# jiahuei/COMIC-Compact-Image-Captioning-with-Attention

Measured on AMD Instinct MI355X. Metric: images/sec (decoder-mode XE training, COMIC-256, InceptionV3 frozen), higher is better.
Workload: dtype bf16; 1 GPU; MS-COCO decoder-mode XE, COMIC-256 (radix-256, 8 heads, tied), InceptionV3 frozen, batch 64/GPU, 224x224x3 (BASELINE configs[1]); per_gpu_batch=64, global_batch=64, image_size=224, feature_map=5x5x2048, decoder_dtype=f32, parallelism=dp1, encoder_group=8, inputs=resident in HBM, 2 distinct image groups in rotation

## Files before the change

### comic-compact-image-captioning-with-attention_amd/_lib.py

```python
import ctypes as C
import os

_HERE = os.path.dirname(os.path.abspath(__file__))
LIB_PATH = os.environ.get('COMIC_HIP_LIB') or os.path.join(_HERE, 'lib', 'libcomic_hip.so')

c_void_p, c_int, c_int32, c_int64, c_float, c_double, c_char_p, c_uint64 = (
    C.c_void_p, C.c_int, C.c_int32, C.c_int64, C.c_float, C.c_double, C.c_char_p, C.c_uint64)


class CnnOp(C.Structure):
    _fields_ = [(n, c_int32) for n in (
        'kind', 'src', 'dst', 'src_coff', 'dst_coff', 'H', 'W', 'Cin', 'Cout', 'KH', 'KW', 'SH', 'SW',
        'PT', 'PL', 'Ho', 'Wo', 'weight', 'relu', 'out_f32', 'src_f32', 'lane', 'tile', 'group', 'flags', 'min_lds')]


class ImageDesc(C.Structure):
    _fields_ = [('offset', C.c_int64), ('in_h', c_int32), ('in_w', c_int32), ('flip', c_int32), ('oy', c_int32),
                ('ox', c_int32), ('sy', C.c_float), ('sx', C.c_float)]


class ConvWeight(C.Structure):
    _fields_ = [('w', c_void_p), ('scale', c_void_p), ('shift', c_void_p), ('w_frag', c_void_p)]


class AttnDesc(C.Structure):
    _fields_ = [(n, c_int32) for n in ('B', 'M', 'D', 'H', 'Cv', 'method', 'prob', 'tied')]


class DecoderDesc(C.Structure):
    _fields_ = [(n, c_int32) for n in (
        'D', 'E', 'A', 'V', 'C', 'Cg', 'H', 'M', 'Cv', 'fm_projection', 'method', 'prob', 'context_layer',
        'init_method', 'start_id', 'end_id')] + [(n, c_float) for n in (
            'keep_in', 'keep_out', 'keep_alpha', 'map_loss_scale')] + [('flags', C.c_uint32),
                                                                       ('length_penalty_weight', c_float),
                                                                       ('cell', c_int32)]


CELLS = {'LSTM': 0, 'LN_LSTM': 1, 'GRU': 2}


(DEC_NO_PERSIST, DEC_NO_PERSIST_BWD, DEC_NO_FUSED_STEP, DEC_NO_SPLIT_ATTN_BWD, DEC_ONE_LANE, DEC_EXACT_GEMM, DEC_STAMPS,
 DEC_NO_BEAM_LOGITS, DEC_NO_LSTM_STREAM) = (1, 2, 4, 8, 16, 32, 64, 128, 256)
DEC_PHASE_FWD, DEC_PHASE_BWD = 512, 1024
DEC_NO_GROUP_GEMM = 2048
DEC_BWD_OWN_ROWS = 4096
DEC_INJECT_TIMEOUT = 8192
CNN_BWD_NO_ACT_FUSION = 2
_DEC_ENV = (('COMIC_PERSIST', '0', DEC_NO_PERSIST), ('COMIC_PERSIST_BWD', '0', DEC_NO_PERSIST_BWD),
            ('COMIC_FUSED_STEP', '0', DEC_NO_FUSED_STEP), ('COMIC_SPLIT_ATTN_BWD', '0', DEC_NO_SPLIT_ATTN_BWD),
            ('COMIC_GRAD_LANES', '0', DEC_ONE_LANE), ('COMIC_SPLIT3', '0', DEC_EXACT_GEMM),
            ('COMIC_PERSIST_STAMPS', '1', DEC_STAMPS), ('COMIC_BEAM_LOGITS', '0', DEC_NO_BEAM_LOGITS),
            ('COMIC_LSTM_STREAM', '0', DEC_NO_LSTM_STREAM), ('COMIC_GROUP_GEMM', '0', DEC_NO_GROUP_GEMM),
            ('COMIC_BWD_OWN_ROWS', '1', DEC_BWD_OWN_ROWS))


def decoder_flags_from_env():
    f = 0
    for name, val, bit in _DEC_ENV:
        if os.environ.get(name, '')[:1] == val:
            f |= bit
    return f


CONV_TILES = 61
WS_TILE = 54
IMG_TILE = 55
CHAIN_TILE = 62
OP_RAW, OP_POOLED_SRC, OP_X3 = 1, 2, 4
OP_CHAIN_LINK = 8
OP_CHAIN_KEEP = 16
IM2COL_CONV_TILES = 12


def is_im2col_tile(tile):
    return tile <= IM2COL_CONV_TILES or 26 <= tile <= 47
PARAM_NAMES = ('W_init', 'K', 'b', 'W_m', 'W_v', 'W_q', 'v', 'ln_g', 'ln_b', 'tau', 'W_a', 'W_o', 'b_o', 'emb', 'cell_ln', 'K_c', 'b_c', 'status')


class DecoderParams(C.Structure):
    _fields_ = [(n, c_void_p) for n in PARAM_NAMES]


class GemmProb(C.Structure):
    _fields_ = [(n, c_void_p) for n in ('A', 'B', 'C', 'bias', 'mask')] + [(n, c_int32) for n in (
        'M', 'N', 'K', 'lda', 'ldb', 'ldc', 'ld_mask')] + [(n, c_float) for n in ('alpha', 'beta', 'keep')] + [
        ('type', c_int32), ('ones_a', c_int32)]


class ConvGrad(C.Structure):
    _fields_ = [('w_master', c_void_p), ('dw', c_void_p), ('dbeta', c_void_p), ('w_bwd', c_void_p),
                ('bwd_tile', c_int32), ('reserved', c_int32)]


P = c_void_p
_SIGS = {
    'comic_last_error': (c_char_p, []),
    'comic_abi_version': (c_int, []),
    'comic_device_count': (c_int, []),
    'comic_pack_conv_weights': (c_int, [P, P, c_int, c_int, c_int, c_int, c_int, P]),
    'comic_fold_bn': (c_int, [P, P, P, c_float, P, P, c_int, P]),
    'comic_cnn_forward': (c_int, [P, c_int, P, P, P, c_int, c_int, P]),
    'comic_cnn_group_args_bytes': (C.c_long, [P, c_int]),
    'comic_cnn_build_group_args': (c_int, [P, c_int, P, P, P, c_int, P]),
    'comic_cnn_forward_grouped': (c_int, [P, c_int, P, P, P, c_int, c_int, P, P]),
    'comic_clip_by_norm': (c_int, [P, P, P, c_int, c_float, c_float, c_float, P, P, P]),
    'comic_cnn_backward_scratch_bytes': (c_int64, [P, c_int, c_int, c_int, c_int]),
    'comic_cnn_backward': (c_int, [P, c_int, P, P, P, P, P, c_int, c_int, c_int, P, c_int64, P, P]),
    'comic_cnn_backward_sched': (c_int, [P, c_int, P, c_int, P, P, P, P, P, P, c_int, c_int, c_int, P, c_int64, P, P, P]),
    'comic_cnn_pack_bwd_filters': (c_int, [P, c_int, P, c_int, P]),
    'comic_cnn_pack_x3_weights': (c_int, [P, P, P, P, P, c_int, P]),
    'comic_cnn_refresh_weights': (c_int, [P, P, c_int64, P, P, P, P, c_int64, P]),
    'comic_cnn_refresh_weights_dtype': (c_int, [P, P, c_int64, P, P, P, P, c_int64, c_int, P]),
    'comic_cnn_pack_frag_weights': (c_int, [P, P, P, c_int, c_int64, P]),
    'comic_crc32c': (C.c_uint32, [P, C.c_size_t, C.c_uint32]),
    'comic_conv2d_bn_relu': (c_int, [P, P, c_int, P, c_int, P, c_int, c_int, P]),
    'comic_gemm_f32': (c_int, [P, P, P, P, c_int, c_int, c_int, c_int, c_int, c_int, c_int, c_int, c_float,
                               c_float, P]),
    'comic_gemm_f32_split3': (c_int, [P, P, P, P, c_int, c_int, c_int, c_int, c_int, c_int, c_int, c_int, c_float,
                                      c_float, P, c_int64, P]),
    'comic_gemm_f32_splitk': (c_int, [P, P, P, P, c_int, c_int, c_int, c_int, c_int, c_int, c_int, c_int, c_float,
                                      c_float, P, c_int64, P]),
    'comic_gemm_group_workspace': (c_int64, [P, c_int]),
    'comic_gemm_group': (c_int, [P, c_int, P, c_int64, P]),
    'comic_embed_fwd': (c_int, [P, P, P, c_int, c_int, c_int, P]),
    'comic_embed_bwd': (c_int, [P, P, P, c_int, c_int, c_int, P]),
    'comic_dropout_apply': (c_int, [P, P, c_float, P, c_int64, P]),
    'comic_dropout_mask': (c_int, [P, c_int64, c_float, c_uint64, c_uint64, P]),
    'comic_dropout_mask_dev': (c_int, [P, c_int64, c_float, P, c_uint64, P]),
    'comic_dropout_masks4_dev': (c_int, [P, P, P, P, P]),
    'comic_image_preprocess': (c_int, [P, P, c_int, P, c_int, c_int, c_int, P]),
    'comic_jpeg_pixels': (c_int, [P, P, c_int, c_int, c_int, c_int, P, P, P]),
    'comic_jpeg_preprocess': (c_int, [P, P, c_int, c_int, P, P, P, P, c_int, c_int, c_int, P]),
    'comic_jpeg_preprocess_packed': (c_int, [P, P, c_int, c_int, P, P, P, P, c_int, c_int, c_int, P]),
    'comic_weighted_sum_tb': (c_int, [P, P, c_int, c_int, P, P]),
    'comic_lstm_gates_fwd': (c_int, [P, P, P, P, P, P, P, P, c_float, P, c_int, P, P, c_int, c_int, P]),
    'comic_lstm_gates_bwd': (c_int, [P, P, P, P, P, c_float, P, c_int, P, P, P, c_int, c_int, P]),
    'comic_attn_step_fwd': (c_int, [P, P, P, P, P, P, P, P, P, c_float, P, P, P, P]),
    'comic_attn_step_bwd': (c_int, [P, P, P, P, P, P, P, P, P, P, c_float, P, P, P, P, P, P, P]),
    'comic_xent_fwd_bwd': (c_int, [P, P, P, P, P, P, P, P, c_int, c_int, c_int, P]),
    'comic_argmax_rows': (c_int, [P, P, c_int, c_int, P]),
    'comic_beam_step': (c_int, [P, P, P, P, P, P, P, c_int, c_int, c_int, c_int, P]),
    'comic_gather_rows': (c_int, [P, P, P, c_int, c_int, c_int, P]),
    'comic_gather_tree': (c_int, [P, P, P, P, c_int, c_int, c_int, c_int, P]),
    'comic_adam_tf': (c_int, [P, P, P, P, c_int64, c_float, c_float, c_float, c_float, c_float, c_float, P]),
    'comic_adam_tf_gated': (c_int, [P, P, P, P, c_int64, c_float, c_float, c_float, c_float, c_float, c_float, P, P]),
    'comic_momentum_tf_gated': (c_int, [P, P, P, c_int64, c_float, c_float, c_float, c_float, P, P]),
    'comic_debug_occupy_cus': (c_int, [c_int, c_int, P]),
    'comic_colsum': (c_int, [P, P, c_int, c_int, c_float, P]),
    'comic_ln_tanh_fwd': (c_int, [P, P, P, P, P, c_int, c_int, c_float, P]),
    'comic_ln_tanh_bwd_rows': (c_int, [P, P, P, P, P, c_int, c_int, P]),
    'comic_momentum_tf': (c_int, [P, P, P, c_int64, c_float, c_float, c_float, c_float, P]),
    'comic_axpy': (c_int, [P, P, c_float, c_int64, P]),
    'comic_decoder_train_workspace': (c_int64, [P, c_int, c_int]),
    'comic_decoder_train_path': (c_int, []),
    'comic_decoder_greedy_path': (c_int, []),
    'comic_decoder_beam_path': (c_int, []),
    'comic_beam_step_dense_workspace': (c_int64, [c_int, c_int, c_int, c_int]),
    'comic_beam_step_dense': (c_int, [c_void_p] * 9 + [c_int] * 5 + [c_void_p, c_int64, c_void_p]),
    'comic_gemm_f32_stream_workspace': (c_int64, [c_int, c_int, c_int]),
    'comic_gemm_f32_stream': (c_int, [c_void_p, c_void_p, c_void_p, c_void_p, c_int, c_int, c_int, c_void_p, c_int64, c_void_p]),
    'comic_decoder_infer_workspace': (c_int64, [P, c_int, c_int]),
    'comic_decoder_train_step': (c_int, [P, P, P, P, P, P, P, P, P, P, c_int, c_int, c_int, P, P, P, P, P, P, P,
                                         P, P, P, P, P, c_int64, P]),
    'comic_decoder_greedy': (c_int, [P, P, P, P, c_int, c_int, P, P, P, P, P, c_int64, P]),
    'comic_decoder_sample': (c_int, [P, P, P, P, c_int, c_int, P, P, P, P, P, P, c_int64, P]),
    'comic_decoder_beam': (c_int, [P, P, P, P, c_int, c_int, c_int, P, P, P, P, P, P, P, P, c_int64, P]),
    'comic_scorer_create': (c_void_p, [c_char_p, P, c_int64, c_double]),
    'comic_scorer_destroy': (None, [c_void_p]),
    'comic_scorer_score': (c_int, [c_void_p, P, c_int, P, P, P, P, c_int]),
}
EXPORTED_SYMBOLS = tuple(_SIGS)

_lib = None


class ComicHipError(RuntimeError):
    pass


def load():
    global _lib
    if _lib is not None:
        return _lib
    if not os.path.exists(LIB_PATH):
        raise ComicHipError(
            'HIP library not built: %s is missing (run `python -c "import __graft_entry__ as g; g.build()"`). '
            'There is no CPU fallback.' % LIB_PATH)
    try:
        import torch
    except ImportError:
        pass
    lib = C.CDLL(LIB_PATH)
    for name, (res, args) in _SIGS.items():
        try:
            fn = getattr(lib, name)
        except AttributeError:
            raise ComicHipError('libcomic_hip.so does not export %s' % name)
        fn.restype = res
        fn.argtypes = args
    if lib.comic_abi_version() != 1:
        raise ComicHipError('ABI version mismatch')
    _lib = lib
    return lib


JPEG_LIB_PATH = os.path.join(os.path.dirname(LIB_PATH), 'libcomic_jpeg.so')
JPEG_OK, JPEG_UNSUPPORTED, JPEG_CORRUPT, JPEG_TOO_SMALL, JPEG_IO = 0, 1, -1, -2, -3


class JpegInfo(C.Structure):
    _fields_ = [('width', C.c_int32), ('height', C.c_int32), ('ncomp', C.c_int32), ('hmax', C.c_int32), ('vmax', C.c_int32),
                ('mcus_x', C.c_int32), ('mcus_y', C.c_int32), ('restart_interval', C.c_int32),
                ('blocks_w', C.c_int32 * 3), ('blocks_h', C.c_int32 * 3), ('comp_w', C.c_int32 * 3), ('comp_h', C.c_int32 * 3),
                ('coef_off', C.c_int64 * 3), ('coef_count', C.c_int64), ('coef_base', C.c_int64), ('pixel_off', C.c_int64),
                ('quant', (C.c_uint16 * 64) * 3)]


JPEG_INFO_DTYPE = [('width', '<i4'), ('height', '<i4'), ('ncomp', '<i4'), ('hmax', '<i4'), ('vmax', '<i4'), ('mcus_x', '<i4'),
                   ('mcus_y', '<i4'), ('restart_interval', '<i4'), ('blocks_w', '<i4', 3), ('blocks_h', '<i4', 3),
                   ('comp_w', '<i4', 3), ('comp_h', '<i4', 3), ('coef_off', '<i8', 3), ('coef_count', '<i8'),
                   ('coef_base', '<i8'), ('pixel_off', '<i8'), ('quant', '<u2', (3, 64))]

_JPEG_SIGS = {
    'comic_jpeg_read_header': (c_int, [P, C.c_int64, P]),
    'comic_jpeg_decode_coefficients': (c_int, [P, C.c_int64, P, P]),
    'comic_jpeg_decode_file': (c_int, [C.c_char_p, P, P, C.c_int64]),
    'comic_jpeg_pool_create': (P, [c_int]),
    'comic_jpeg_pool_destroy': (None, [P]),
    'comic_jpeg_pool_submit': (P, [P, P, c_int, P, P, P, C.c_int64]),
    'comic_jpeg_pool_submit_packed': (P, [P, P, c_int, P, P, P, C.c_int64]),
    'comic_jpeg_pool_wait': (c_int, [P, P, C.c_double, P, P]),
    'comic_jpeg_pool_enable_cache': (c_int, [P, C.c_int64]),
    'comic_jpeg_pool_cache_stats': (c_int, [P, P, P, P]),
}
JPEG_EXPORTED_SYMBOLS = tuple(_JPEG_SIGS)
_jpeg_lib = None


def load_jpeg():
    global _jpeg_lib
    if _jpeg_lib is not None:
        return _jpeg_lib
    if not os.path.exists(JPEG_LIB_PATH):
        raise ComicHipError('JPEG entropy library not built: %s is missing (run `make -C csrc`)' % JPEG_LIB_PATH)
    assert C.sizeof(JpegInfo) == 512
    lib = C.CDLL(JPEG_LIB_PATH)
    for name, (res, args) in _JPEG_SIGS.items():
        try:
            fn = getattr(lib, name)
        except AttributeError:
            raise ComicHipError('libcomic_jpeg.so does not export %s' % name)
        fn.restype = res
        fn.argtypes = args
    _jpeg_lib = lib
    return lib


def check(rc, what=''):
    if rc != 0:
        msg = load().comic_last_error()
        raise ComicHipError('%s failed (rc=%d): %s' % (what or 'comic_hip call', rc, msg.decode() if msg else ''))


def ptr(t):
    if t is None:
        return None
    assert t.is_contiguous(), 'tensor must be contiguous'
    return t.data_ptr()


def stream_ptr():
    import torch
    return torch.cuda.current_stream().cuda_stream
```

### comic-compact-image-captioning-with-attention_amd/csrc/decoder_exec.hip

```cpp
#include <atomic>
#include <stdlib.h>

#include <algorithm>
#include <string.h>

#include "common.h"
#include "decoder_math.h"
#include "decoder_persist.h"
#include "gemm_group.h"
#include "lstm_prep.h"
#include "lstm_stream_dev.h"

int comic_gemm_f32_ws(const float* A, const float* B, float* C, const float* bias, int M, int N, int K, int lda,
                      int ldb, int ldc, int trans_a, int trans_b, float alpha, float beta, void* ws, int64_t ws_bytes,
                      hipStream_t st);
int comic_xent_ex(float* logits, const int32_t* targets_bt, const float* coef_bt, const float* wmask_bt,
                  const int32_t* lens, float* loss_rows, float* dlogits, int32_t* ids_tb, int t_rows, int t_stride,
                  int B, int V, hipStream_t st);

int comic_attn_fwd_ex(const comic_attn_desc* d, const float* keys, const float* values, const float* q,
                      const float* ln_g, const float* ln_b, const float* v, const float* tau, const float* mask_alpha,
                      float keep_alpha, float* alpha, float* alpha_d, float* ctx, const int32_t* lens, int t,
                      const float* att_prev, float* att_next, float* xh_next, int xh_ld, const float* mask_next,
                      int mask_ld, float keep_in, int q_parts, float* q_out, float* scores_ws, hipStream_t st,
// ... 242 lines not shown
  if (i < n_x) {
    const long r = i / E;
    const int e = (int)(i % E), t = (int)(r / B), b = (int)(r % B);
    const int id = ids_bt[(size_t)b * T + t];
    if (e == 0) ids_tb[r] = id;
    float v = (id >= 0 && id < V) ? table[(size_t)id * E + e] : 0.f;
    if (mask) v = (v / keep) * mask[(size_t)r * EA + e];
    xh[(size_t)r * Wd + e] = v;
  } else if (i < n_x + (long)B * A) {
    const long j = i - n_x;
    att0[j] = 0.f;
    xh[(size_t)(j / A) * Wd + E + (j % A)] = 0.f;
  } else if (i < n_x + (long)B * A + (long)B * D) {
    const long j = i - n_x - (long)B * A;
    float hv;
    if (cell_g) {
      const int b = (int)(j / D), dd = (int)(j % D);
      const float* gr = cell_g + (size_t)b * 4 * D;
      const float si = sigmoidf_(gr[dd]), tj = tanhf(gr[D + dd]);
      const float sf = sigmoidf_(gr[2 * D + dd] + 1.0f), so = sigmoidf_(gr[3 * D + dd]);
      const float c2 = 0.f * sf + si * tj;
      hv = tanhf(c2) * so;
      float* ga = cell_gates + (size_t)b * 4 * D;
      ga[dd] = si; ga[D + dd] = tj; ga[2 * D + dd] = sf; ga[3 * D + dd] = so;
      cell_cnew[j] = c2;
      c0[j] = c2;
      h0_out[j] = hv;
    } else {
      hv = h0[j];
    }
    xh[(size_t)(j / D) * Wd + EA + (j % D)] = hv;
  } else if (xh_init && i < n_x + (long)B * A + 2L * B * D) {
    const long j = i - n_x - (long)B * A - (long)B * D;
    xh_init[(size_t)(j / D) * Wd + EA + (j % D)] = 0.f;
  }
}

__global__ void infer_prep_kernel(const float* __restrict__ table, const int32_t* __restrict__ ids,
                                  const int32_t* __restrict__ parent, int W, const float* __restrict__ att,
                                  const float* __restrict__ h, const float* __restrict__ c, float* __restrict__ xh,
                                  float* __restrict__ c_in, int R, int E, int A, int D, int V,
                                  const int32_t* __restrict__ stop, int stop_t) {
  if (comic_stopped(stop, stop_t)) return;
  const int Wd = E + A + D, cols = Wd + D;
  const long i = (long)blockIdx.x * blockDim.x + threadIdx.x;
  if (i >= (long)R * cols) return;
  const int r = (int)(i / cols), k = (int)(i % cols);
  const int src = parent ? (r / W) * W + min(max(parent[r], 0), W - 1) : r;
  if (k < E) {
    const int id = ids[r];
    xh[(size_t)r * Wd + k] = (id >= 0 && id < V) ? table[(size_t)id * E + k] : 0.f;
  } else if (k < E + A) {
    xh[(size_t)r * Wd + k] = att[(size_t)src * A + (k - E)];
  } else if (k < Wd) {
    xh[(size_t)r * Wd + k] = h[(size_t)src * D + (k - E - A)];
  } else {
    c_in[(size_t)r * D + (k - Wd)] = c[(size_t)src * D + (k - Wd)];
  }
}

__global__ void select_att_kernel(const float* __restrict__ prev, const float* __restrict__ cur,
                                  const int32_t* __restrict__ lens, int t, float* __restrict__ dst,
                                  float* __restrict__ xh_next, int xh_ld, const float* __restrict__ mask_next,
                                  int mask_ld, float keep, int B, int A) {
  const int i = blockIdx.x * blockDim.x + threadIdx.x;
  if (i >= B * A) return;
  const int b = i / A, c = i % A;
  const float v = (lens && t >= lens[b]) ? prev[i] : cur[i];
  dst[i] = v;
  if (xh_next) {
    float x = v;
    if (mask_next) x = (x / keep) * mask_next[(size_t)b * mask_ld + c];
    xh_next[(size_t)b * xh_ld + c] = x;
  }
}

__global__ void select_rows_kernel(const float* __restrict__ prev, const float* __restrict__ cur,
                                   const int32_t* __restrict__ lens, int t, float* __restrict__ dst, int B, int C) {
  const int i = blockIdx.x * blockDim.x + threadIdx.x;
  if (i >= B * C) return;
  const int b = i / C;
  dst[i] = (lens && t >= lens[b]) ? prev[i] : cur[i];
}

__global__ void split_live_kernel(float* __restrict__ d, float* __restrict__ out_live,
                                  const int32_t* __restrict__ lens, int t, int B, int C) {
  const int i = blockIdx.x * blockDim.x + threadIdx.x;
  if (i >= B * C) return;
  const int b = i / C;
  const bool fin = lens && t >= lens[b];
  const float v = d[i];
  out_live[i] = fin ? 0.f : v;
  d[i] = fin ? v : 0.f;
}

__global__ void input_bwd_kernel(const float* __restrict__ dxh, const float* __restrict__ mask, float keep,
                                 float* __restrict__ demb, float* __restrict__ datt, float* __restrict__ dh,
                                 const int32_t* __restrict__ lens, int t, int carry, int B, int E, int A, int D,
                                 int S) {
  const int W = E + A + D;
  const int i = blockIdx.x * blockDim.x + threadIdx.x;
  if (i >= B * W) return;
  const int b = i / W, c = i % W;
  float v = dxh[i];
  for (int s = 1; s < S; ++s) v += dxh[(size_t)s * B * W + i];
  if (c < E + A) {
    if (mask) v = (v / keep) * mask[(size_t)b * (E + A) + c];
    if (c < E) {
      if (demb) demb[(size_t)b * E + c] = v;
    } else {
      float* p = datt + (size_t)b * A + (c - E);
      const bool fin = lens && t >= lens[b];
      *p = ((carry && !fin) ? 0.f : *p) + v;
    }
  } else {
    dh[(size_t)b * D + (c - E - A)] += v;
  }
}

__global__ __launch_bounds__(256) void maploss_part_kernel(const float* __restrict__ hist, float* __restrict__ dmap,
                                                           float* __restrict__ partial, int Tp, int B, int H, int M,
                                                           float scale) {
  __shared__ float red[256];
  const long n = (long)Tp * B * M;
  const long i = (long)blockIdx.x * 256 + threadIdx.x;
  float acc = 0.f;
  if (i < n) {
    const int m = (int)(i % M);
    const long tb = i / M;
    const float* p = hist + (size_t)tb * H * M + m;
    float f = 0.f;
    for (int h = 0; h < H; ++h) f += p[(size_t)h * M];
    const float d = 1.0f - f;
    acc = d * d;
    if (dmap) dmap[i] = 2.0f * (f - 1.0f) / (float)n * scale;
  }
  red[threadIdx.x] = acc;
  __syncthreads();
  for (int s = 128; s > 0; s >>= 1) {
    if (threadIdx.x < s) red[threadIdx.x] += red[threadIdx.x + s];
    __syncthreads();
  }
  if (threadIdx.x == 0) partial[blockIdx.x] = red[0];
}
__global__ void scatter_pgrad_kernel(const float* __restrict__ row, float* __restrict__ v, float* __restrict__ ln_g,
                                     float* __restrict__ ln_b, float* __restrict__ tau, int D) {
  const int i = blockIdx.x * blockDim.x + threadIdx.x;
  if (i < D) {
    v[i] = row[i];
    ln_g[i] = row[D + i];
    ln_b[i] = row[2 * D + i];
  }
  if (i == 0) tau[0] = row[3 * D];
}

__global__ __launch_bounds__(256) void maploss_final_kernel(const float* __restrict__ partial, int nparts, long n,
                                                            float scale, float* __restrict__ map_loss) {
  __shared__ float red[256];
  float acc = 0.f;
  for (int i = threadIdx.x; i < nparts; i += 256) acc += partial[i];
  red[threadIdx.x] = acc;
  __syncthreads();
  for (int s = 128; s > 0; s >>= 1) {
    if (threadIdx.x < s) red[threadIdx.x] += red[threadIdx.x + s];
    __syncthreads();
  }
  if (threadIdx.x == 0) map_loss[0] = red[0] / (float)n * scale;
}

__global__ __launch_bounds__(1024) void maploss_kernel(const float* __restrict__ hist, float* __restrict__ dmap,
                                                       float* __restrict__ map_loss, int Tp, int B, int H, int M,
                                                       float scale) {
  __shared__ float red[1024];
  const long n = (long)Tp * B * M;
  float acc = 0.f;
  for (long i = threadIdx.x; i < n; i += 1024) {
    const int m = (int)(i % M);
    const long tb = i / M;
    const float* p = hist + (size_t)tb * H * M + m;
    float f = 0.f;
    for (int h = 0; h < H; ++h) f += p[(size_t)h * M];
    const float d = 1.0f - f;
    acc += d * d;
    if (dmap) dmap[i] = 2.0f * (f - 1.0f) / (float)n * scale;
  }
  red[threadIdx.x] = acc;
  __syncthreads();
  for (int s = 512; s > 0; s >>= 1) {
    if (threadIdx.x < s) red[threadIdx.x] += red[threadIdx.x + s];
    __syncthreads();
  }
  if (threadIdx.x == 0 && map_loss) map_loss[0] = red[0] / (float)n * scale;
}

__global__ void fill_kernel(float* p, float v, long n) {
  const long i = (long)blockIdx.x * blockDim.x + threadIdx.x;
  if (i < n) p[i] = v;
}
__global__ void fill_i32_kernel(int32_t* p, int32_t v, long n) {
  const long i = (long)blockIdx.x * blockDim.x + threadIdx.x;
  if (i < n) p[i] = v;
}
__global__ void transpose_ids_kernel(const int32_t* __restrict__ in_bt, int32_t* __restrict__ out_tb, int B, int T,
                                     int Tp) {
  const int i = blockIdx.x * blockDim.x + threadIdx.x;
  if (i >= Tp * B) return;
  const int t = i / B, b = i % B;
  out_tb[i] = in_bt[(size_t)b * T + t];
}
__global__ void tile_rows_kernel(const float* __restrict__ in, float* __restrict__ out, long total, int W, int cols) {
  const long i = (long)blockIdx.x * blockDim.x + threadIdx.x;
  if (i >= total) return;
  const long r = i / cols;
  out[i] = in[(size_t)(r / W) * cols + (i % cols)];
}
__global__ void eos_track_done_kernel(const int32_t* __restrict__ ids, int32_t* __restrict__ first_eos, int t,
                                      int end_id, int B, int32_t* __restrict__ steps_done, int max_steps) {
  __shared__ int any_live;
  if (threadIdx.x == 0) any_live = 0;
  __syncthreads();
  if (steps_done[0] <= t) return;
  for (int b = threadIdx.x; b < B; b += blockDim.x) {
    int fe = first_eos[b];
    if (ids[b] == end_id && fe > t) {
      fe = t;
      first_eos[b] = t;
    }
    if (fe > t) any_live = 1;
  }
  __syncthreads();
  if (threadIdx.x == 0 && !any_live && steps_done[0] == max_steps) steps_done[0] = t + 1;
}
__global__ void all_finished_kernel(const int32_t* __restrict__ finished, int32_t* __restrict__ steps_executed, int t,
                                    int n, int max_steps) {
  __shared__ int any_live;
  if (threadIdx.x == 0) any_live = 0;
  __syncthreads();
  for (int i = threadIdx.x; i < n; i += blockDim.x)
    if (!finished[i]) any_live = 1;
  __syncthreads();
  if (threadIdx.x == 0 && !any_live && steps_executed[0] == max_steps) steps_executed[0] = t + 1;
}

__global__ void beam_init_kernel(float* __restrict__ log_probs, int32_t* __restrict__ finished,
                                 int64_t* __restrict__ lengths, int R, int W) {
  const int i = blockIdx.x * blockDim.x + threadIdx.x;
  if (i >= R) return;
  const bool first = (i % W) == 0;
  log_probs[i] = first ? 0.f : -INFINITY;
  finished[i] = first ? 0 : 1;
  lengths[i] = 0;
}

__global__ void pad_rows_kernel(const float* __restrict__ in, float* __restrict__ out, int cols, int ld, long n) {
  const long i = (long)blockIdx.x * blockDim.x + threadIdx.x;
  if (i >= n) return;
  const long r = i / ld;
  const int c = (int)(i - r * ld);
  out[i] = c < cols ? in[r * cols + c] : 0.f;
}

inline int fill(float* p, float v, long n, hipStream_t st) {
  if (n <= 0) return 0;
  hipLaunchKernelGGL(fill_kernel, dim3((unsigned)cdiv64(n, 256)), dim3(256), 0, st, p, v, n);
  COMIC_LAUNCH_CHECK("fill");
  return 0;
}
constexpr int64_t kSplitKBytes = 32ll << 20;

inline int gemm(const float* A, const float* B, float* C, const float* bias, int M, int N, int K, int lda, int ldb,
                int ldc, int ta, int tb, float beta, hipStream_t st) {
  return comic_gemm_f32_ws(A, B, C, bias, M, N, K, lda, ldb, ldc, ta, tb, 1.0f, beta, g_splitk_ws,
                           g_splitk_ws ? kSplitKBytes : 0, st);
}

inline int gemm_big(const float* A, const float* B, float* C, const float* bias, int M, int N, int K, int lda, int ldb,
                    int ldc, int ta, int tb, float beta, hipStream_t st) {
  const bool on = !(g_dec_flags & COMIC_DEC_EXACT_GEMM);
  if (!on || (long)M * N < 64 * 256 || K < 64)
    return gemm(A, B, C, bias, M, N, K, lda, ldb, ldc, ta, tb, beta, st);
  return comic_gemm_bf16x3_impl(A, B, C, bias, M, N, K, lda, ldb, ldc, ta, tb, 1.0f, beta, g_splitk_ws,
                                g_splitk_ws ? kSplitKBytes : 0, st);
}

constexpr int kGroupTickets = 4096;
struct GemmGroupRun {
  ComicGemmGroup g{};
  ComicGemmProb* add(int type, const float* A, const float* B, float* C, int M, int N, int K, int lda, int ldb, int ldc) {
    if (g.n >= kGemmGroupMax) return nullptr;
    ComicGemmProb& p = g.p[g.n++];
    p = ComicGemmProb{};
    p.type = type; p.A = A; p.B = B; p.C = C; p.M = M; p.N = N; p.K = K; p.lda = lda; p.ldb = ldb; p.ldc = ldc;
    p.alpha = 1.f; p.beta = 0.f; p.keep = 1.f;
    return &p;
  }
  ComicGemmProb* add_colsum(const float* B, float* C, int N, int K, int ldb) {
    ComicGemmProb* p = add(COMIC_GG_TN, nullptr, B, C, 1, N, K, 1, ldb, N);
    if (p) p->ones_a = 1;
    return p;
  }
  int run(void* slab, int64_t slab_cap, unsigned* tickets, hipStream_t st) {
    if (g.n == 0) return 0;
    int target = kGemmGroupTargetItems;
    for (;;) {
      int64_t need = 0;
      int nt = 0;
      const int wg = comic_gemm_group_plan(g, target, &need, &nt);
      if (wg < 0) return 2;
      if (need <= slab_cap && nt <= kGroupTickets - 8) {
        g.slab = (float*)slab;
        g.tickets = tickets;
        return comic_gemm_group_launch(g, wg, st);
      }
      COMIC_REQUIRE(target > 1, "gemm_group: split-K scratch too small");
      target = target / 2;
    }
  }
};

int check_desc(const comic_decoder_desc* d) {
  COMIC_REQUIRE(d, "decoder: null descriptor");
  COMIC_REQUIRE(d->D > 0 && d->E > 0 && d->A > 0 && d->V > 1 && d->C > 0 && d->Cg > 0 && d->H > 0 && d->M > 0,
                "decoder: bad dimensions");
  const int cv = d->fm_projection == 0 ? d->C : d->D;
  COMIC_REQUIRE(d->Cv == cv, "decoder: Cv must be %d for fm_projection %d", cv, d->fm_projection);
  const int a = (d->fm_projection == 0 && !d->context_layer) ? d->C : d->D;
  COMIC_REQUIRE(d->A == a, "decoder: attention size A must be %d", a);
  COMIC_REQUIRE(d->cell >= COMIC_CELL_LSTM && d->cell <= COMIC_CELL_GRU, "decoder: unknown cell %d", d->cell);
  return 0;
}
int check_cell_params(const comic_decoder_desc* d, const comic_decoder_params* p) {
  COMIC_REQUIRE(p && p->K, "decoder: null cell kernel");
  if (d->cell == COMIC_CELL_LSTM) COMIC_REQUIRE(p->b, "decoder: LSTM needs its bias");
  if (d->cell == COMIC_CELL_LN_LSTM) COMIC_REQUIRE(p->cell_ln, "decoder: LN_LSTM needs cell_ln");
  if (d->cell == COMIC_CELL_GRU) COMIC_REQUIRE(p->b && p->K_c && p->b_c, "decoder: GRU needs b, K_c, b_c");
  return 0;
}

comic_attn_desc attn_desc(const comic_decoder_desc* d, int rows) {
  comic_attn_desc a;
  a.B = rows; a.M = d->M; a.D = d->D; a.H = d->H; a.Cv = d->Cv;
  a.method = d->method; a.prob = d->prob; a.tied = d->fm_projection == 2;
  return a;
}

int memory_projections(const comic_decoder_desc* d, const comic_decoder_params* p, const float* fm, int rows,
                       float* keys, float* values_buf, const float** values, hipStream_t st) {
  RC(gemm_big(fm, p->W_m, keys, nullptr, rows * d->M, d->D, d->C, d->C, d->D, d->D, 0, 0, 0.f, st));
  if (d->fm_projection == 2) {
    *values = keys;
  } else if (d->fm_projection == 1) {
    RC(gemm_big(fm, p->W_v, values_buf, nullptr, rows * d->M, d->D, d->C, d->C, d->D, d->D, 0, 0, 0.f, st));
    *values = values_buf;
  } else {
    *values = fm;
  }
  return 0;
}

struct InitBufs {
  float *x, *xh, *g, *gates, *c_new;
  float *lnx = nullptr, *lnr = nullptr;
};

int rnn_init_fwd(const comic_decoder_desc* d, const comic_decoder_params* p, const float* im_embed, int rows,
                 const float* mask_init, InitBufs& ib, float* c0, float* h0, hipStream_t st) {
  const int D = d->D, EA = d->E + d->A;
  if (d->init_method == 1) {
    RC(gemm(im_embed, p->W_init, h0, nullptr, rows, D, d->Cg, d->Cg, D, D, 0, 0, 0.f, st));
    RC(fill(c0, 0.f, (long)rows * D, st));
    return 0;
  }
  RC(gemm(im_embed, p->W_init, ib.x, nullptr, rows, EA, d->Cg, d->Cg, EA, EA, 0, 0, 0.f, st));
  RC(comic_dropout_apply(ib.x, mask_init, d->keep_in, ib.xh, (int64_t)rows * EA, (void*)st));
  if (d->cell == COMIC_CELL_LN_LSTM) {
    RC(gemm(ib.xh, p->K, ib.g, nullptr, rows, 4 * D, EA, EA, 4 * D, 4 * D, 0, 0, 0.f, st));
    return comic_ln_lstm_fwd(ib.g, 1, p->cell_ln, nullptr, nullptr, ib.gates, ib.lnx, ib.lnr, ib.c_new, nullptr, nullptr, 1.f,
                             nullptr, 0, c0, h0, rows, D, nullptr, 0, st);
  }
  if (d->cell == COMIC_CELL_GRU) {
    float* g2 = ib.g + (size_t)rows * 2 * D;
    RC(gemm(ib.xh, p->K, ib.g, nullptr, rows, 2 * D, EA, EA, 2 * D, 2 * D, 0, 0, 0.f, st));
    RC(comic_gru_gates_fwd(ib.g, 1, p->b, nullptr, ib.xh, EA, ib.gates, 4 * D, nullptr, 0, rows, D, EA, st));
    RC(gemm(ib.xh, p->K_c, g2, nullptr, rows, D, EA, EA, D, D, 0, 0, 0.f, st));
    RC(comic_gru_out_fwd(g2, 1, p->b_c, ib.gates, 4 * D, nullptr, ib.gates + 2 * D, 4 * D, nullptr, nullptr, 1.f, nullptr, 0,
                         h0, nullptr, 0, rows, D, st));
    return fill(c0, 0.f, (long)rows * D, st);
  }
  RC(gemm(ib.xh, p->K, ib.g, p->b, rows, 4 * D, EA, EA, 4 * D, 4 * D, 0, 0, 0.f, st));
  RC(comic_lstm_gates_fwd(ib.g, nullptr, nullptr, ib.gates, ib.c_new, nullptr, nullptr, nullptr, 1.f, nullptr, 0, c0,
                          h0, rows, D, (void*)st));
  return 0;
}

struct StepBufs {
  float *xh, *g, *y, *q, *alpha, *ctx, *c2, *h2, *att2;
  float* xh2 = nullptr;
};
int infer_step(const comic_decoder_desc* d, const comic_decoder_params* p, const comic_attn_desc& ad,
               const float* keys, const float* values, const float* x, const float* c, const float* h,
               const float* att, StepBufs& sb, float* alpha_d_out, int rows, hipStream_t st) {
  const int D = d->D, E = d->E, A = d->A, Wd = E + A + D;
  hipLaunchKernelGGL(assemble_input_kernel, dim3(cdiv(rows * Wd, 256)), dim3(256), 0, st, x, att, h, nullptr, 1.f,
                     sb.xh, rows, E, A, D);
  COMIC_LAUNCH_CHECK("assemble_input");
  if (d->cell == COMIC_CELL_LN_LSTM) {
    RC(gemm(sb.xh, p->K, sb.g, nullptr, rows, 4 * D, Wd, Wd, 4 * D, 4 * D, 0, 0, 0.f, st));
    RC(comic_ln_lstm_fwd(sb.g, 1, p->cell_ln, c, h, nullptr, nullptr, nullptr, nullptr, sb.y, nullptr, 1.f, nullptr, 0, sb.c2,
                         sb.h2, rows, D, nullptr, 0, st));
  } else if (d->cell == COMIC_CELL_GRU) {
    float* ru = sb.g + (size_t)rows * 2 * D;
    RC(gemm(sb.xh, p->K, sb.g, nullptr, rows, 2 * D, Wd, Wd, 2 * D, 2 * D, 0, 0, 0.f, st));
    RC(comic_gru_gates_fwd(sb.g, 1, p->b, h, sb.xh, Wd, ru, 2 * D, sb.xh2, Wd, rows, D, E + A, st));
    RC(gemm(sb.xh2, p->K_c, sb.q, nullptr, rows, D, Wd, Wd, D, D, 0, 0, 0.f, st));
    RC(comic_gru_out_fwd(sb.q, 1, p->b_c, ru, 2 * D, h, nullptr, 0, sb.y, nullptr, 1.f, nullptr, 0, sb.h2, nullptr, 0, rows, D,
                         st));
    RC(fill(sb.c2, 0.f, (long)rows * D, st));
  } else {
    RC(gemm(sb.xh, p->K, sb.g, p->b, rows, 4 * D, Wd, Wd, 4 * D, 4 * D, 0, 0, 0.f, st));
    RC(comic_lstm_gates_fwd(sb.g, c, h, nullptr, nullptr, nullptr, sb.y, nullptr, 1.f, nullptr, 0, sb.c2, sb.h2, rows,
                            D, (void*)st));
  }
  RC(gemm(sb.y, p->W_q, sb.q, nullptr, rows, D, D, D, D, D, 0, 0, 0.f, st));
  RC(comic_attn_step_fwd(&ad, keys, values, sb.q, p->ln_g, p->ln_b, p->v, p->tau, nullptr, 1.f, sb.alpha,
                         alpha_d_out, sb.ctx, (void*)st));
  if (d->context_layer) {
    RC(gemm(sb.ctx, p->W_a, sb.att2, nullptr, rows, D, d->Cv, d->Cv, D, D, 0, 0, 0.f, st));
  }
  return 0;
}

struct StreamBufs {
  const void* kfrag;
  void* xfrag;
  void* yfrag;
  const void* wqfrag;
  int skip_prep = 0;
  const void* wofrag = nullptr;
  int wo_N = 0;
  float* wo_part = nullptr;
  int wo_S = 0;
  int q_S = 0;
};
int infer_step_lstm(const comic_decoder_desc* d, const comic_decoder_params* p, const float* kpanel, const int32_t* ids,
                    const int32_t* parent, int W, const float* c_src, const float* h_src, const float* att_src,
                    StepBufs& sb, float* c_in, int rows, hipStream_t st, const StreamBufs* sm) {
  const int D = d->D, E = d->E, A = d->A, Wd = E + A + D;
  if (sm) {
    RC(comic_lstm_stream_step(p->emb, ids, parent, W, att_src, h_src, c_src, sm->kfrag, p->b, sm->xfrag, c_in,
                              (float*)g_splitk_ws, kSplitKBytes, sb.c2, sb.h2, sb.y, sm->yfrag, rows, E, A, D, d->V, sm->skip_prep, st));
  } else {
    const long n = (long)rows * (Wd + D);
    hipLaunchKernelGGL(infer_prep_kernel, dim3((unsigned)cdiv64(n, 256)), dim3(256), 0, st, p->emb, ids, parent, W,
                       att_src, h_src, c_src, sb.xh, c_in, rows, E, A, D, d->V, g_comic_stop.p, g_comic_stop.t);
    COMIC_LAUNCH_CHECK("infer_prep");
    RC(comic_lstm_step_fused(sb.xh, Wd, kpanel, p->b, c_in, nullptr, nullptr, nullptr, sb.y, nullptr, 1.f, nullptr, 0,
                             sb.c2, sb.h2, nullptr, 0, rows, D, Wd, st));
  }
  return 0;
}
int infer_step_attend(const comic_decoder_desc* d, const comic_decoder_params* p, const comic_attn_desc& ad,
                      const float* keys, const float* values, StepBufs& sb, float* alpha_d_out, int rows, hipStream_t st,
                      StreamBufs* sm, int mem_div) {
  const int D = d->D;
  int S = 1;
  float* part = (float*)g_splitk_ws;
  if (sm && sm->q_S > 0) {
    S = sm->q_S;
  } else if (sm && sm->wqfrag && sm->wofrag) {
    sm->wo_part = (float*)((char*)g_splitk_ws + kSplitKBytes / 2);
    RC(comic_stream_gemm2(sm->yfrag, sm->wqfrag, part, D, &S, sm->wofrag, sm->wo_part, sm->wo_N, &sm->wo_S, kSplitKBytes / 2,
                          rows, D, st));
  } else if (sm && sm->wqfrag) RC(comic_stream_gemm(sm->yfrag, sm->wqfrag, part, kSplitKBytes, rows, D, D, &S, st));
  else RC(comic_gemm_f32_partial(sb.y, p->W_q, rows, D, D, D, D, 0, part, kSplitKBytes, &S, st));
  float* attn_ws = ((long)d->H * d->M <= 4L * D) ? sb.g : nullptr;
  RC(comic_attn_fwd_ex(&ad, keys, values, part, p->ln_g, p->ln_b, p->v, p->tau, nullptr, 1.f, sb.alpha, alpha_d_out,
                       sb.ctx, nullptr, 0, nullptr, nullptr, nullptr, 0, nullptr, 0, 1.f, S, nullptr, attn_ws, st, mem_div));
  if (d->context_layer) {
    RC(gemm(sb.ctx, p->W_a, sb.att2, nullptr, rows, D, d->Cv, d->Cv, D, D, 0, 0, 0.f, st));
  }
  return 0;
}
int infer_step_fused(const comic_decoder_desc* d, const comic_decoder_params* p, const comic_attn_desc& ad,
                     const float* keys, const float* values, const float* kpanel, const int32_t* ids,
                     const int32_t* parent, int W, const float* c_src, const float* h_src, const float* att_src,
                     StepBufs& sb, float* c_in, float* alpha_d_out, int rows, hipStream_t st,
                     StreamBufs* sm = nullptr, int mem_div = 1) {
  RC(infer_step_lstm(d, p, kpanel, ids, parent, W, c_src, h_src, att_src, sb, c_in, rows, st, sm));
  return infer_step_attend(d, p, ad, keys, values, sb, alpha_d_out, rows, st, sm, mem_div);
}

}

thread_local int g_train_path = 0;
extern "C" int comic_decoder_train_path(void) { return g_train_path; }
thread_local int g_greedy_path = 0;
extern "C" int comic_decoder_greedy_path(void) { return g_greedy_path; }
thread_local int g_beam_path = 0;
extern "C" int comic_decoder_beam_path(void) { return g_beam_path; }

extern "C" int64_t comic_decoder_train_workspace(const comic_decoder_desc* d, int B, int T) {
  if (!d) return -1;
  Bump w(nullptr, 0);
  const long D = d->D, E = d->E, A = d->A, V = d->V, M = d->M, H = d->H, Cv = d->Cv, Wd = E + A + D;
  const long TB = (long)T * B;
  w.take<float>(B * M * D); w.take<float>(B * M * D);
  w.take<float>(B * (E + A)); w.take<float>(B * (E + A));
  w.take<float>(B * 4 * D); w.take<float>(B * 4 * D); w.take<float>(B * D);
  w.take<float>(TB * E); w.take<int32_t>(TB);
  w.take<float>((TB + B) * Wd); w.take<float>(B * 4 * D);
  w.take<float>(TB * 4 * D);
  w.take<float>((TB + B) * D); w.take<float>((TB + B) * D);
  w.take<float>(TB * D); w.take<float>(TB * D); w.take<float>(TB * D);
  w.take<float>(TB * H * M);
  w.take<float>(TB * Cv); w.take<float>(B * D); w.take<float>((TB + B) * A);
  w.take<float>(TB * ((V + 3) / 4 * 4));
  w.take<float>(D * ((V + 3) / 4 * 4));
  w.take<float>(TB * D); w.take<float>(TB * D); w.take<float>((TB + B) * 4 * D);
  w.take<float>(B * Wd); w.take<float>(B * D); w.take<float>(B * D);
  w.take<float>(B * A); w.take<float>(B * A); w.take<float>(B * Cv);
  w.take<float>(TB * E); w.take<float>(B * M * D); w.take<float>(B * M * Cv);
  w.take<float>(TB * (3 * D + 1)); w.take<float>(TB * M);
  w.take<float>(B * (E + A));
  w.take<char>(kSplitKBytes);
  w.take<char>(kSplitKBytes);
  w.take<float>(comic_lstm_panel_floats((int)D, (int)Wd, 0));
  w.take<float>(comic_lstm_panel_floats((int)D, (int)Wd, 1));
  w.take<float>(D * D);
  w.take<unsigned>(kPersistSyncWords + kGroupTickets);
  w.take<float>(TB * 4 * D); w.take<float>((long)T * ((B + 15) / 16) * 16 * 4 * D);
  w.take<float>((long)T * ((B + 15) / 16) * 16 * D);
  w.take<float>(TB * 2 * D);
  w.take<float>(4 * B * (3 * D + 1));
  w.take<float>(TB * 64);
  if (comic_persist_fwd_bigm((int)M, d->fm_projection == 2)) w.take<float>(TB * 8 * M);
  if (d->cell == COMIC_CELL_LN_LSTM) {
    w.take<float>((TB + B) * 5 * D); w.take<float>((TB + B) * 8); w.take<float>((TB + B) * 10 * D); w.take<float>(10 * D);
  } else if (d->cell == COMIC_CELL_GRU) {
    w.take<float>(TB * Wd); w.take<float>(2 * B * Wd); w.take<float>(4 * D);
  }
  return (int64_t)w.off;
}

extern "C" int comic_decoder_train_step(const comic_decoder_desc* d, const comic_decoder_params* p,
                                        const comic_decoder_params* gr, const float* fm, const float* im_embed,
                                        const int32_t* inputs_bt, const int32_t* targets_bt, const float* wmask_bt,
                                        const float* coef_bt, const int32_t* lens, int B, int T, int Tp,
                                        const float* mask_init_in, const float* mask_in, const float* mask_out,
                                        const float* mask_alpha, float* logits_tb, int32_t* ids_tb, float* attn_hist,
                                        float* loss_rows, float* map_loss, float* dfm, float* dim_embed,
                                        void* workspace, int64_t workspace_bytes, void* stream) {
  RC(check_desc(d));
  FlagScope flag_scope__(d);
  COMIC_REQUIRE(p && gr && fm && im_embed && inputs_bt && targets_bt && wmask_bt && coef_bt && lens,
                "train_step: null input");
  COMIC_REQUIRE(logits_tb && ids_tb && attn_hist && loss_rows && map_loss && workspace, "train_step: null output");
  COMIC_REQUIRE(B > 0 && T > 0 && Tp > 0 && Tp <= T, "train_step: bad B/T/Tp (%d %d %d)", B, T, Tp);
  COMIC_REQUIRE(workspace_bytes >= comic_decoder_train_workspace(d, B, T), "train_step: workspace too small");
  COMIC_REQUIRE(d->keep_in >= 1.f || (mask_in && (d->init_method == 1 || mask_init_in)),
                "train_step: input dropout enabled but no mask given");
  COMIC_REQUIRE(d->keep_out >= 1.f || mask_out, "train_step: output dropout enabled but no mask given");
  COMIC_REQUIRE(d->keep_alpha >= 1.f || mask_alpha, "train_step: attention dropout enabled but no mask given");
  hipStream_t st = (hipStream_t)stream;
  const int D = d->D, E = d->E, A = d->A, V = d->V, M = d->M, H = d->H, Cv = d->Cv, EA = E + A, Wd = E + A + D;
  const long TB = (long)T * B;
  const bool drop_in = d->keep_in < 1.f, drop_out = d->keep_out < 1.f, drop_al = d->keep_alpha < 1.f;
  Bump w(workspace, (size_t)workspace_bytes);
  float* keys = w.take<float>((long)B * M * D);
  float* values_buf = w.take<float>((long)B * M * D);
  InitBufs ib;
  ib.x = w.take<float>((long)B * EA); ib.xh = w.take<float>((long)B * EA);
  ib.g = w.take<float>((long)B * 4 * D); ib.gates = w.take<float>((long)B * 4 * D); ib.c_new = w.take<float>((long)B * D);
  float* emb_all = w.take<float>(TB * E);
  int32_t* in_tb = w.take<int32_t>(TB);
  float* xh_all = w.take<float>((TB + B) * Wd);
  float* g_tmp = w.take<float>((long)B * 4 * D);
  float* gates_all = w.take<float>(TB * 4 * D);
  float* cs = w.take<float>((TB + B) * D);
  float* hs = w.take<float>((TB + B) * D);
  float* cnew_all = w.take<float>(TB * D);
  float* y_all = w.take<float>(TB * D);
  float* q_all = w.take<float>(TB * D);
  float* alpha_all = w.take<float>(TB * H * M);
  float* ctx_all = w.take<float>(TB * Cv);
  float* att_new = w.take<float>((long)B * D);
  float* att_all = w.take<float>((TB + B) * A);
  const int Vp = (V + 3) / 4 * 4;
  float* dlogits = w.take<float>(TB * Vp);
  float* wo_pad = w.take<float>((long)D * Vp);
  float* dy_all = w.take<float>(TB * D);
  float* dq_all = w.take<float>(TB * D);
  float* dg_all = w.take<float>((TB + B) * 4 * D);
  float* dxh = w.take<float>((long)B * Wd);
  float* dc = w.take<float>((long)B * D);
  float* dh = w.take<float>((long)B * D);
  float* datt = w.take<float>((long)B * A);
  float* datt_live = w.take<float>((long)B * A);
  float* dctx = w.take<float>((long)B * Cv);
  float* demb = w.take<float>(TB * E);
  float* dkeys = w.take<float>((long)B * M * D);
  float* dvalues_buf = w.take<float>((long)B * M * Cv);
  float* pgrad = w.take<float>(TB * (3 * D + 1));
  float* dmap = w.take<float>(TB * M);
  float* dx_init = w.take<float>((long)B * EA);
  g_splitk_ws = w.take<char>(kSplitKBytes);
  void* splitk_ws_b = w.take<char>(kSplitKBytes);
// ... 934 lines not shown
```

### comic-compact-image-captioning-with-attention_amd/csrc/gemm_group.h

```cpp
#pragma once
#include "common.h"

constexpr int kGemmGroupMax = 20;
enum { COMIC_GG_TN = 0, COMIC_GG_NN = 1, COMIC_GG_NT = 2 };

struct ComicGemmProb {
  const float* A;
  const float* B;
  float* C;
  const float* bias;
  const float* mask;
  int M, N, K, lda, ldb, ldc, ld_mask;
  float alpha, beta;
  float keep;
  int type;
  int ones_a;
  int tiles_m, tiles_n, S, k_per_slice, wg_begin;
  int slab_tile0;
  int ticket0;
};

struct ComicGemmGroup {
  ComicGemmProb p[kGemmGroupMax];
  int n;
  float* slab;
  unsigned* tickets;
  int xcd_chunk;
};

int comic_gemm_group_plan(ComicGemmGroup& g, int target_items, int64_t* slab_bytes, int* n_tickets);
constexpr int kGemmGroupTargetItems = 640;
int comic_gemm_group_launch(const ComicGemmGroup& g, int n_wg, hipStream_t st);
```

### comic-compact-image-captioning-with-attention_amd/csrc/gemm_group.hip

```cpp
#include <algorithm>

#include "gemm_group.h"
#include "gemm_x3_dev.h"

namespace {

constexpr int GB = 128;
constexpr int kGemmGroupSlots = 512;
constexpr int kItemOverhead = 6;
constexpr int kSc1 = 16;
typedef __attribute__((ext_vector_type(4))) unsigned gg_u32x4_t;

__device__ __forceinline__ __amdgpu_buffer_rsrc_t gg_rsrc(const void* p, long bytes) {
  return __builtin_amdgcn_make_buffer_rsrc((void*)p, 0, (int)bytes, 0x00020000);
}
__device__ __forceinline__ float4 gg_load16_sc1(__amdgpu_buffer_rsrc_t r, unsigned off) {
  const gg_u32x4_t v = __builtin_amdgcn_raw_buffer_load_b128(r, (int)off, 0, kSc1);
  return make_float4(__uint_as_float(v.x), __uint_as_float(v.y), __uint_as_float(v.z), __uint_as_float(v.w));
}
__device__ __forceinline__ void gg_store16_sc1(__amdgpu_buffer_rsrc_t r, unsigned off, float4 v) {
  const gg_u32x4_t u = {__float_as_uint(v.x), __float_as_uint(v.y), __float_as_uint(v.z), __float_as_uint(v.w)};
  __builtin_amdgcn_raw_buffer_store_b128(u, r, (int)off, 0, kSc1);
}

constexpr int kGroupLds = 4 * (X3Tile<GB, true>::BYTES + X3Tile<GB, true>::BYTES);
static_assert(X3Tile<GB, true>::BYTES >= X3Tile<GB, false>::BYTES, "LDS of the k-contiguous form bounds the others");
constexpr int kGroupLdsPc = 2 * 2 * (X3TilePc<GB, false>::BYTES + X3TilePc<GB, false>::BYTES);
static_assert(X3TilePc<GB, false>::BYTES >= X3TilePc<GB, true>::BYTES, "LDS of the row-contiguous form bounds the others");

__device__ __forceinline__ void gg_emit(const ComicGemmProb& p, int m, int n, float4 a) {
  if (m >= p.M || n >= p.N) return;
  const int nv = min(4, p.N - n);
  float v[4] = {a.x * p.alpha, a.y * p.alpha, a.z * p.alpha, a.w * p.alpha};
  float* cp = p.C + (size_t)m * p.ldc + n;
#pragma unroll
  for (int q = 0; q < 4; ++q) {
    if (q >= nv) break;
    if (p.bias) v[q] += p.bias[n + q];
    if (p.mask) v[q] = (v[q] / p.keep) * p.mask[(size_t)m * p.ld_mask + n + q];
    if (p.beta != 0.f) v[q] += p.beta * cp[q];
  }
  if (nv == 4 && (p.ldc % 4 == 0) && (((uintptr_t)p.C & 15) == 0)) {
    *(float4*)cp = make_float4(v[0], v[1], v[2], v[3]);
  } else {
#pragma unroll
    for (int q = 0; q < 4; ++q)
      if (q < nv) cp[q] = v[q];
  }
}

template <bool PC>
__global__ __launch_bounds__(PC ? 512 : 256) void gemm_group_x3_kernel(ComicGemmGroup g) {
  constexpr int NT = PC ? 512 : 256;
  constexpr int LDS = PC ? kGroupLdsPc : kGroupLds;
  extern __shared__ __attribute__((aligned(16))) unsigned char smem[];
  int bid = blockIdx.x;
  if (g.xcd_chunk > 0 && bid < g.xcd_chunk * 8) bid = (bid & 7) * g.xcd_chunk + (bid >> 3);
  volatile unsigned* s_last = (volatile unsigned*)(smem + LDS - 16);
  int pi = 0;
#pragma unroll 1
  for (int i = 1; i < g.n; ++i)
    if (bid >= g.p[i].wg_begin) pi = i;
  const ComicGemmProb& p = g.p[pi];
  const int local = bid - p.wg_begin;
  const int S = p.S, ntiles = p.tiles_m * p.tiles_n;
  const int slice = local / ntiles, tl = local - slice * ntiles;
  constexpr int PW = 8;
  const int panel = tl / (p.tiles_m * PW), rem = tl - panel * p.tiles_m * PW;
  const int pw = min(PW, p.tiles_n - panel * PW);
  const int mt = rem / pw, nt = panel * PW + rem % pw;
  const int tile = mt * p.tiles_n + nt;
  const int m0 = mt * GB, n0 = nt * GB;
  const int kbeg = S > 1 ? slice * p.k_per_slice : 0;
  const int kend = S > 1 ? min(p.K, kbeg + p.k_per_slice) : p.K;
  const int tid = threadIdx.x, lane = tid & 63, wave = tid >> 6;
  const int wm = wave >> 1, wn = wave & 1;

  const long tile_id = (long)p.ticket0 + tile;
  const __amdgpu_buffer_rsrc_t sr = gg_rsrc(g.slab + ((long)p.slab_tile0 + (long)tile * S) * (GB * GB), (long)S * GB * GB * 4);
  const unsigned sbase = (unsigned)slice * (GB * GB * 4);
  if (p.ones_a) {
    constexpr int KG = NT / 32;
    float4* red = (float4*)smem;
    const int cg = tid & 31, kg = tid >> 5, n = n0 + 4 * cg;
    const bool vec = (p.ldb % 4 == 0) && (((uintptr_t)p.B & 15) == 0);
    float4 sm = make_float4(0.f, 0.f, 0.f, 0.f);
    if (n < p.N)
      for (int k = kbeg + kg; k < kend; k += KG) {
        const float4 v = load4(p.B + (size_t)k * p.ldb + n, p.N - n, vec);
        sm.x += v.x; sm.y += v.y; sm.z += v.z; sm.w += v.w;
      }
    red[kg * 32 + cg] = sm;
    __syncthreads();
    if (tid < 32) {
      float4 tot = red[cg];
#pragma unroll
      for (int k = 1; k < KG; ++k) {
        const float4 v = red[k * 32 + cg];
        tot.x += v.x; tot.y += v.y; tot.z += v.z; tot.w += v.w;
      }
      if (S == 1) gg_emit(p, 0, n, tot);
      else gg_store16_sc1(sr, sbase + (unsigned)cg * 16u, tot);
    }
    if (S == 1) return;
  } else {
    f32x4_t acc[4][4];
    if constexpr (PC) {
      if (p.type == COMIC_GG_TN) x3_mainloop_pc<false, false>(p.A, p.B, p.M, p.N, p.lda, p.ldb, m0, n0, kbeg, kend, smem, acc);
      else if (p.type == COMIC_GG_NN) x3_mainloop_pc<true, false>(p.A, p.B, p.M, p.N, p.lda, p.ldb, m0, n0, kbeg, kend, smem, acc);
      else x3_mainloop_pc<true, true>(p.A, p.B, p.M, p.N, p.lda, p.ldb, m0, n0, kbeg, kend, smem, acc);
    } else {
      if (p.type == COMIC_GG_TN)
        x3_mainloop<GB, false, false, GB>(p.A, p.B, p.M, p.N, p.lda, p.ldb, m0, n0, kbeg, kend, smem, acc);
      else if (p.type == COMIC_GG_NN)
        x3_mainloop<GB, true, false, GB>(p.A, p.B, p.M, p.N, p.lda, p.ldb, m0, n0, kbeg, kend, smem, acc);
      else
        x3_mainloop<GB, true, true, GB>(p.A, p.B, p.M, p.N, p.lda, p.ldb, m0, n0, kbeg, kend, smem, acc);
    }
    const bool owner = wave < 4;
    if (S == 1) {
      if (owner)
#pragma unroll
      for (int i = 0; i < 4; ++i)
#pragma unroll
        for (int j = 0; j < 4; ++j)
          gg_emit(p, m0 + wm * 64 + j * 16 + (lane & 15), n0 + wn * 64 + i * 16 + (lane >> 4) * 4,
                  make_float4(acc[i][j][0], acc[i][j][1], acc[i][j][2], acc[i][j][3]));
      return;
    }
    if (owner)
#pragma unroll
    for (int i = 0; i < 4; ++i)
#pragma unroll
      for (int j = 0; j < 4; ++j) {
        const int ml = wm * 64 + j * 16 + (lane & 15), nl = wn * 64 + i * 16 + (lane >> 4) * 4;
        gg_store16_sc1(sr, sbase + (unsigned)(ml * GB + nl) * 4u, make_float4(acc[i][j][0], acc[i][j][1], acc[i][j][2], acc[i][j][3]));
      }
  }
  asm volatile("s_waitcnt vmcnt(0)" ::: "memory");
  __syncthreads();
  if (tid == 0) {
    const unsigned t = __hip_atomic_fetch_add(g.tickets + tile_id, 1u, __ATOMIC_RELAXED, __HIP_MEMORY_SCOPE_AGENT);
    *s_last = (t == (unsigned)(S - 1)) ? 1u : 0u;
    if (t == (unsigned)(S - 1)) __hip_atomic_store(g.tickets + tile_id, 0u, __ATOMIC_RELAXED, __HIP_MEMORY_SCOPE_AGENT);
  }
  __syncthreads();
  if (!*s_last) return;
  const int n_chunks = p.ones_a ? 1 : (GB * GB / 4) / NT;
#pragma unroll 1
  for (int c = 0; c < n_chunks; c += 4) {
    float4 sum[4];
#pragma unroll
    for (int u = 0; u < 4; ++u) sum[u] = make_float4(0.f, 0.f, 0.f, 0.f);
#pragma unroll 1
    for (int s = 0; s < S; ++s) {
      float4 v[4];
#pragma unroll
      for (int u = 0; u < 4; ++u) v[u] = gg_load16_sc1(sr, (unsigned)s * (GB * GB * 4) + (unsigned)(tid + NT * (c + u)) * 16u);
#pragma unroll
      for (int u = 0; u < 4; ++u) {
        sum[u].x += v[u].x; sum[u].y += v[u].y; sum[u].z += v[u].z; sum[u].w += v[u].w;
      }
    }
#pragma unroll
    for (int u = 0; u < 4; ++u) {
      const int idx4 = tid + NT * (c + u);
      if (!p.ones_a || idx4 < GB / 4) gg_emit(p, m0 + idx4 / (GB / 4), n0 + (idx4 % (GB / 4)) * 4, sum[u]);
    }
  }
}


}

int comic_gemm_group_plan(ComicGemmGroup& g, int target_items, int64_t* slab_bytes, int* n_tickets) {
  COMIC_REQUIRE(g.n > 0 && g.n <= kGemmGroupMax, "gemm_group: %d problems", g.n);
  long cost = 0;
  for (int i = 0; i < g.n; ++i) {
    ComicGemmProb& p = g.p[i];
    COMIC_REQUIRE(p.M > 0 && p.N > 0 && p.K > 0 && p.B && p.C && (p.A || p.ones_a), "gemm_group: bad problem %d", i);
    COMIC_REQUIRE(p.type >= COMIC_GG_TN && p.type <= COMIC_GG_NT, "gemm_group: bad type of problem %d", i);
    COMIC_REQUIRE(!p.ones_a || (p.type == COMIC_GG_TN && p.M == 1), "gemm_group: ones_a needs type TN and M = 1 (problem %d)", i);
    COMIC_REQUIRE(p.ldc >= p.N && (!p.mask || p.ld_mask >= p.N), "gemm_group: leading dimension of problem %d", i);
    if (!p.ones_a) COMIC_REQUIRE(p.lda >= (p.type == COMIC_GG_TN ? p.M : p.K), "gemm_group: lda of problem %d", i);
    COMIC_REQUIRE(p.ldb >= (p.type == COMIC_GG_NT ? p.K : p.N), "gemm_group: ldb of problem %d", i);
    p.tiles_m = cdiv(p.M, GB);
    p.tiles_n = cdiv(p.N, GB);
    cost += (long)cdiv(p.M, GB) * p.tiles_n * cdiv(p.K, 32);
  }
  auto split_of = [](int kt, long klen) { return (int)std::min<long>(16, std::max<long>(1, (kt + klen / 2) / klen)); };
  long klen = std::max<long>(8, cost / std::max(1, target_items));
  {
    long best = -1, best_klen = klen, kt_max = 8;
    for (int i = 0; i < g.n; ++i) kt_max = std::max<long>(kt_max, cdiv(g.p[i].K, 32));
    for (long kl = klen; kl <= kt_max; ++kl) {
      long items = 0, longest = 0;
      for (int i = 0; i < g.n; ++i) {
        const ComicGemmProb& p = g.p[i];
        const int kt = cdiv(p.K, 32), S = split_of(kt, kl);
        items += (long)p.tiles_m * p.tiles_n * S;
        if (!p.ones_a) longest = std::max<long>(longest, cdiv(kt, S));
      }
      const long est = cdiv64(items, kGemmGroupSlots) * (longest + kItemOverhead);
      if (best < 0 || est < best) {
        best = est;
        best_klen = kl;
      }
    }
    klen = best_klen;
  }
  int wg = 0, tickets = 0, slab_tiles = 0;
  for (int i = 0; i < g.n; ++i) {
    ComicGemmProb& p = g.p[i];
    const int nt = cdiv(p.M, GB) * p.tiles_n, kt = cdiv(p.K, 32);
    int S = split_of(kt, klen);
    p.k_per_slice = cdiv(kt, S) * 32;
    S = cdiv(p.K, p.k_per_slice);
    p.S = S;
    p.wg_begin = wg;
    p.slab_tile0 = slab_tiles;
    p.ticket0 = tickets;
    wg += nt * S;
    if (S > 1) {
      slab_tiles += nt * S;
      tickets += nt;
    }
  }
  if (slab_bytes) *slab_bytes = (int64_t)slab_tiles * GB * GB * 4;
  if (n_tickets) *n_tickets = tickets;
  return wg;
}

int comic_gemm_group_launch(const ComicGemmGroup& g_in, int n_wg, hipStream_t st) {
  ComicGemmGroup g = g_in;
  g.xcd_chunk = n_wg / 8;
  COMIC_REQUIRE(n_wg > 0, "gemm_group: empty launch");
  bool pc = n_wg <= 256;
  for (int i = 0; i < g.n && pc; ++i) {
    const ComicGemmProb& p = g.p[i];
    if (p.ones_a) continue;
    const bool a_kc = p.type != COMIC_GG_TN, b_kc = p.type == COMIC_GG_NT;
    pc = p.lda % 4 == 0 && p.ldb % 4 == 0 && ((uintptr_t)p.A & 15) == 0 && ((uintptr_t)p.B & 15) == 0 &&
         (!(a_kc || b_kc) || p.K % 4 == 0);
  }
  static PerDeviceOnce once, once_pc;
  bool& done = pc ? once_pc.slot() : once.slot();
  const int lds = pc ? kGroupLdsPc : kGroupLds;
  if (!done) {
    const void* fn = pc ? (const void*)gemm_group_x3_kernel<true> : (const void*)gemm_group_x3_kernel<false>;
    COMIC_REQUIRE(hipFuncSetAttribute(fn, hipFuncAttributeMaxDynamicSharedMemorySize, lds) == hipSuccess,
                  "gemm_group: cannot reserve %d bytes of LDS", lds);
    done = true;
  }
  if (pc) hipLaunchKernelGGL(gemm_group_x3_kernel<true>, dim3((unsigned)n_wg), dim3(512), lds, st, g);
  else hipLaunchKernelGGL(gemm_group_x3_kernel<false>, dim3((unsigned)n_wg), dim3(256), lds, st, g);
  COMIC_LAUNCH_CHECK("gemm_group");
  return 0;
}

namespace {
int gg_from_public(const comic_gemm_prob* probs, int n, ComicGemmGroup& g) {
  COMIC_REQUIRE(probs && n > 0 && n <= kGemmGroupMax, "gemm_group: 1..%d problems", kGemmGroupMax);
  g = ComicGemmGroup{};
  g.n = n;
  for (int i = 0; i < n; ++i) {
    const comic_gemm_prob& q = probs[i];
    ComicGemmProb& p = g.p[i];
    p.A = q.A; p.B = q.B; p.C = q.C; p.bias = q.bias; p.mask = q.mask;
    p.M = q.M; p.N = q.N; p.K = q.K; p.lda = q.lda; p.ldb = q.ldb; p.ldc = q.ldc; p.ld_mask = q.ld_mask;
    p.alpha = q.alpha; p.beta = q.beta; p.keep = q.keep; p.type = q.type; p.ones_a = q.ones_a;
  }
  return 0;
}
#define kPublicTarget kGemmGroupTargetItems
}

extern "C" int64_t comic_gemm_group_workspace(const comic_gemm_prob* probs, int n) {
  ComicGemmGroup g;
  if (gg_from_public(probs, n, g)) return -1;
  int64_t slab = 0;
  int nt = 0;
  if (comic_gemm_group_plan(g, kPublicTarget, &slab, &nt) < 0) return -1;
  return slab + 256 + (int64_t)nt * 4;
}

extern "C" int comic_gemm_group(const comic_gemm_prob* probs, int n, void* workspace, int64_t workspace_bytes, void* stream) {
  ComicGemmGroup g;
  if (int rc = gg_from_public(probs, n, g)) return rc;
  int64_t slab = 0;
  int nt = 0;
  const int wg = comic_gemm_group_plan(g, kPublicTarget, &slab, &nt);
  if (wg < 0) return 2;
  const int64_t slab_al = (slab + 255) / 256 * 256;
  COMIC_REQUIRE(nt == 0 || (workspace && workspace_bytes >= slab_al + (int64_t)nt * 4), "gemm_group: workspace too small");
  g.slab = (float*)workspace;
  g.tickets = nt ? (unsigned*)((char*)workspace + slab_al) : nullptr;
  if (nt) COMIC_REQUIRE(hipMemsetAsync(g.tickets, 0, (size_t)nt * 4, (hipStream_t)stream) == hipSuccess, "gemm_group: memset");
  return comic_gemm_group_launch(g, wg, (hipStream_t)stream);
}
```

### comic-compact-image-captioning-with-attention_amd/csrc/gemm_x3_dev.h

```cpp
#pragma once
#include <type_traits>

#include "common.h"

namespace {

__device__ __forceinline__ float4 load4(const float* __restrict__ p, int nvalid, bool vec_ok) {
  if (nvalid >= 4 && vec_ok) return *(const float4*)p;
  float4 r = make_float4(0.f, 0.f, 0.f, 0.f);
  if (nvalid > 0) r.x = p[0];
  if (nvalid > 1) r.y = p[1];
  if (nvalid > 2) r.z = p[2];
  if (nvalid > 3) r.w = p[3];
  return r;
}

__device__ __forceinline__ void split_bf16x2(float a, float b, uint32_t& hi, uint32_t& lo) {
  hi = pack_bf16x2(a, b);
  lo = pack_bf16x2(a - __uint_as_float(hi << 16), b - __uint_as_float(hi & 0xFFFF0000u));
}

template <int ROWS, bool KC>
struct X3Tile {
  static constexpr int ROWB = 80;
  static constexpr int KSTR = 2 * ROWS + 32;
  static constexpr int BYTES = KC ? ROWS * ROWB : 32 * KSTR;
};

template <int ROWS, bool KC>
__device__ __forceinline__ void x3_chunk(int q, int ld, int row0, int rows_total, int k0, int K, int& c, int& ext, int& nv,
                                         size_t& base) {
  int r, k;
  if (KC) {
    r = row0 + (q >> 3); k = k0 + (q & 7) * 4;
    c = k; ext = K; nv = r < rows_total ? K - k : 0;
    base = (size_t)min(r, rows_total - 1) * ld;
  } else {
    constexpr int CPR = ROWS / 4;
    k = k0 + q / CPR; r = row0 + (q % CPR) * 4;
    c = r; ext = rows_total; nv = k < K ? rows_total - r : 0;
    base = (size_t)min(k, K - 1) * ld;
  }
}
template <int ROWS, bool KC, int NCH, bool VEC>
__device__ __forceinline__ void x3_load_tile(const float* __restrict__ g, int ld, int row0, int rows_total, int k0, int K,
                                             int tid, float4 (&out)[NCH]) {
#pragma unroll
  for (int i = 0; i < NCH; ++i) {
    int c, ext, nv;
    size_t base;
    x3_chunk<ROWS, KC>(tid + 256 * i, ld, row0, rows_total, k0, K, c, ext, nv, base);
    const float* bp = g + base;
    if (VEC) {
      out[i] = *(const float4*)(bp + max(0, min(c, ext - 4)));
    } else {
      const int e = ext - 1;
      out[i] = make_float4(bp[min(c, e)], bp[min(c + 1, e)], bp[min(c + 2, e)], bp[min(c + 3, e)]);
    }
  }
}
template <int ROWS, bool KC, int NCH, bool VEC>
__device__ __forceinline__ void x3_mask_tile(int row0, int rows_total, int k0, int K, int tid, float4 (&v)[NCH]) {
#pragma unroll
  for (int i = 0; i < NCH; ++i) {
    int c, ext, nv;
    size_t base;
    x3_chunk<ROWS, KC>(tid + 256 * i, 0, row0, rows_total, k0, K, c, ext, nv, base);
    if (VEC) {
      const bool ok = nv >= 4;
      v[i].x = ok ? v[i].x : 0.f; v[i].y = ok ? v[i].y : 0.f; v[i].z = ok ? v[i].z : 0.f; v[i].w = ok ? v[i].w : 0.f;
    } else {
      v[i].x = nv > 0 ? v[i].x : 0.f; v[i].y = nv > 1 ? v[i].y : 0.f; v[i].z = nv > 2 ? v[i].z : 0.f; v[i].w = nv > 3 ? v[i].w : 0.f;
    }
  }
}
template <int ROWS, bool KC, int NCH>
__device__ __forceinline__ void x3_store_tile(unsigned char* hi_base, unsigned char* lo_base, int tid,
                                              const float4 (&in)[NCH]) {
  using T = X3Tile<ROWS, KC>;
#pragma unroll
  for (int i = 0; i < NCH; ++i) {
    const int q = tid + 256 * i;
    uint32_t h0, l0, h1, l1;
    split_bf16x2(in[i].x, in[i].y, h0, l0);
    split_bf16x2(in[i].z, in[i].w, h1, l1);
    int off;
    if (KC) {
      const int row = q >> 3, c = q & 7;
      off = row * T::ROWB + (2 * (c & 3) + (c >> 2)) * 8;
    } else {
      constexpr int CPR = ROWS / 4;
      const int kk = q / CPR, row = (q % CPR) * 4;
      off = kk * T::KSTR + row * 2;
    }
    *(uint2*)(hi_base + off) = make_uint2(h0, h1);
    *(uint2*)(lo_base + off) = make_uint2(l0, l1);
  }
}
typedef __attribute__((ext_vector_type(4))) short x3_s16x4_t;
typedef __attribute__((ext_vector_type(8))) short x3_s16x8_t;
template <int ROWS, bool KC>
__device__ __forceinline__ bf16x8_t x3_frag(const unsigned char* base, int row16, int lane) {
  using T = X3Tile<ROWS, KC>;
  if (KC) {
    const uint4 v = *(const uint4*)(base + (row16 + (lane & 15)) * T::ROWB + (lane >> 4) * 16);
    return __builtin_bit_cast(bf16x8_t, v);
  } else {
    const int g = lane >> 4, q = (lane >> 2) & 3, pp = lane & 3;
    const unsigned char* p = base + (4 * g + q) * T::KSTR + (row16 + 4 * pp) * 2;
    const uint32_t a0 = (uint32_t)(uintptr_t)((__attribute__((address_space(3))) const unsigned char*)p);
    const x3_s16x4_t lo = __builtin_amdgcn_ds_read_tr16_b64_v4i16((__attribute__((address_space(3))) x3_s16x4_t*)(uintptr_t)a0);
    const x3_s16x4_t hi =
        __builtin_amdgcn_ds_read_tr16_b64_v4i16((__attribute__((address_space(3))) x3_s16x4_t*)(uintptr_t)(a0 + 16 * T::KSTR));
    const x3_s16x8_t v = {lo[0], lo[1], lo[2], lo[3], hi[0], hi[1], hi[2], hi[3]};
    return __builtin_bit_cast(bf16x8_t, v);
  }
}


constexpr unsigned kOor = 0x80000000u;
template <int ROWS, bool KC, int NCH, bool VEC>
struct X3Src {
  const float* g;
  int ld, row0, rows_total, kend;
  __amdgpu_buffer_rsrc_t rs;
  unsigned base;
  unsigned rb[NCH];
  int kc;
  unsigned step8;
  __device__ __forceinline__ void init(const float* g_, int ld_, int row0_, int rows_total_, int kbeg, int kend_, int tid) {
    g = g_; ld = ld_; row0 = row0_; rows_total = rows_total_; kend = kend_;
    if (VEC) {
      rs = __builtin_amdgcn_make_buffer_rsrc((void*)g, 0, 0x7FFFFFF0, 0x00020000);
      if (KC) {
        kc = (tid & 7) * 4;
#pragma unroll
        for (int i = 0; i < NCH; ++i) {
          const int r = row0 + (tid >> 3) + 32 * i;
          rb[i] = r < rows_total ? (unsigned)(((long)r * ld + kc) * 4) : kOor;
        }
      } else {
        constexpr int CPR = ROWS / 4;
        const int r = row0 + (tid % CPR) * 4;
        const long rec = ((long)(kend - 1) * ld + min(ld, (rows_total + 3) & ~3)) * 4;
        rs = __builtin_amdgcn_make_buffer_rsrc((void*)g, 0, (int)rec, 0x00020000);
        base = r < rows_total ? (unsigned)(((long)(kbeg + tid / CPR) * ld + r) * 4) : kOor;
        step8 = (unsigned)((256 / CPR) * ld * 4);
      }
    }
  }
  __device__ __forceinline__ void load(int k0, int tid, float4 (&out)[NCH]) {
    if (VEC) {
      typedef __attribute__((ext_vector_type(4))) unsigned u4;
      if (KC) {
        const unsigned past = (unsigned)((kend - 1 - (k0 + kc)) >> 31) & kOor;
#pragma unroll
        for (int i = 0; i < NCH; ++i) {
          const unsigned o = (rb[i] + (unsigned)k0 * 4u) | past;
          const u4 v = __builtin_amdgcn_raw_buffer_load_b128(rs, (int)o, 0, 0);
          out[i] = make_float4(__uint_as_float(v.x), __uint_as_float(v.y), __uint_as_float(v.z), __uint_as_float(v.w));
        }
      } else if constexpr (256 % (ROWS / 4) == 0) {
#pragma unroll
        for (int i = 0; i < NCH; ++i) {
          const u4 v = __builtin_amdgcn_raw_buffer_load_b128(rs, (int)(base + (unsigned)i * step8), 0, 0);
          out[i] = make_float4(__uint_as_float(v.x), __uint_as_float(v.y), __uint_as_float(v.z), __uint_as_float(v.w));
        }
        base += (unsigned)(32 * ld * 4);
      } else {
        constexpr int CPR = ROWS / 4;
#pragma unroll
        for (int i = 0; i < NCH; ++i) {
          const int q = tid + 256 * i, r = row0 + (q % CPR) * 4;
          const unsigned o = r < rows_total ? (unsigned)(((long)(k0 + q / CPR) * ld + r) * 4) : kOor;
          const u4 v = __builtin_amdgcn_raw_buffer_load_b128(rs, (int)o, 0, 0);
          out[i] = make_float4(__uint_as_float(v.x), __uint_as_float(v.y), __uint_as_float(v.z), __uint_as_float(v.w));
        }
      }
    } else {
      x3_load_tile<ROWS, KC, NCH, false>(g, ld, row0, rows_total, k0, kend, tid, out);
    }
  }
  __device__ __forceinline__ void mask(int k0, int tid, float4 (&v)[NCH]) {
    if (!VEC) x3_mask_tile<ROWS, KC, NCH, false>(row0, rows_total, k0, kend, tid, v);
  }
};

template <int BM, bool A_KC, bool B_KC, int BN, bool VEC>
__device__ __forceinline__ void x3_mainloop_v(const float* __restrict__ A, const float* __restrict__ B, int M, int N, int lda,
                                            int ldb, int m0, int n0, int kbeg, int kend, unsigned char* smem,
                                            f32x4_t (&acc)[BN / 32][BM / 32]) {
  constexpr int BKx = 32;
  constexpr int TM = BM / 32, TN = BN / 32;
  constexpr int ACH = BM * BKx / 4 / 256, BCH = BN * BKx / 4 / 256;
  constexpr int ABYTES = X3Tile<BM, A_KC>::BYTES, BBYTES = X3Tile<BN, B_KC>::BYTES;
  unsigned char* Ah = smem;
  unsigned char* Al = Ah + 2 * ABYTES;
  unsigned char* Bh = Al + 2 * ABYTES;
  unsigned char* Bl = Bh + 2 * BBYTES;
  const int tid = threadIdx.x, lane = tid & 63, wave = tid >> 6;
  const int wm = wave >> 1, wn = wave & 1;
#pragma unroll
  for (int i = 0; i < TN; ++i)
#pragma unroll
    for (int j = 0; j < TM; ++j) acc[i][j] = (f32x4_t){0.f, 0.f, 0.f, 0.f};
  float4 ar[2][ACH], br[2][BCH];
  const int nk = ((kend - kbeg + BKx - 1) / BKx + 1) & ~1;
  X3Src<BM, A_KC, ACH, VEC> sa;
  X3Src<BN, B_KC, BCH, VEC> sb;
  sa.init(A, lda, m0, M, kbeg, kend, tid);
  sb.init(B, ldb, n0, N, kbeg, kend, tid);
  sa.load(kbeg, tid, ar[0]);
  sb.load(kbeg, tid, br[0]);
  sa.load(kbeg + BKx, tid, ar[1]);
  sb.load(kbeg + BKx, tid, br[1]);
  sa.mask(kbeg, tid, ar[0]);
  sb.mask(kbeg, tid, br[0]);
  x3_store_tile<BM, A_KC, ACH>(Ah, Al, tid, ar[0]);
  x3_store_tile<BN, B_KC, BCH>(Bh, Bl, tid, br[0]);
  __syncthreads();
  auto step = [&](const int kt, auto par) {
    constexpr int P = decltype(par)::value;
    sa.load(kbeg + (kt + 2) * BKx, tid, ar[P]);
    sb.load(kbeg + (kt + 2) * BKx, tid, br[P]);
    bf16x8_t bh[TN], bl[TN], ah[TM], al[TM];
#pragma unroll
    for (int i = 0; i < TN; ++i) {
      bh[i] = x3_frag<BN, B_KC>(Bh + P * BBYTES, wn * (BN / 2) + i * 16, lane);
      bl[i] = x3_frag<BN, B_KC>(Bl + P * BBYTES, wn * (BN / 2) + i * 16, lane);
    }
#pragma unroll
    for (int j = 0; j < TM; ++j) {
      ah[j] = x3_frag<BM, A_KC>(Ah + P * ABYTES, wm * (BM / 2) + j * 16, lane);
      al[j] = x3_frag<BM, A_KC>(Al + P * ABYTES, wm * (BM / 2) + j * 16, lane);
    }
#pragma unroll
    for (int i = 0; i < TN; ++i)
#pragma unroll
      for (int j = 0; j < TM; ++j) {
        acc[i][j] = __builtin_amdgcn_mfma_f32_16x16x32_bf16(bl[i], ah[j], acc[i][j], 0, 0, 0);
        acc[i][j] = __builtin_amdgcn_mfma_f32_16x16x32_bf16(bh[i], al[j], acc[i][j], 0, 0, 0);
        acc[i][j] = __builtin_amdgcn_mfma_f32_16x16x32_bf16(bh[i], ah[j], acc[i][j], 0, 0, 0);
      }
    sa.mask(kbeg + (kt + 1) * BKx, tid, ar[P ^ 1]);
    sb.mask(kbeg + (kt + 1) * BKx, tid, br[P ^ 1]);
    x3_store_tile<BM, A_KC, ACH>(Ah + (P ^ 1) * ABYTES, Al + (P ^ 1) * ABYTES, tid, ar[P ^ 1]);
    x3_store_tile<BN, B_KC, BCH>(Bh + (P ^ 1) * BBYTES, Bl + (P ^ 1) * BBYTES, tid, br[P ^ 1]);
#ifdef COMIC_X3_SCHED
    __builtin_amdgcn_sched_group_barrier(0x020, ACH + BCH, 0);
    __builtin_amdgcn_sched_group_barrier(0x100, 64, 0);
#pragma unroll
    for (int r = 0; r < TM * TN; ++r) {
      __builtin_amdgcn_sched_group_barrier(0x008, 3, 0);
      __builtin_amdgcn_sched_group_barrier(0x002, 9, 0);
      __builtin_amdgcn_sched_group_barrier(0x200, 1, 0);
    }
#endif
    __syncthreads();
  };
  for (int kt = 0; kt < nk; kt += 2) {
    step(kt, std::integral_constant<int, 0>());
    step(kt + 1, std::integral_constant<int, 1>());
  }
}

template <int BM, bool A_KC, bool B_KC, int BN>
__device__ __forceinline__ void x3_mainloop(const float* __restrict__ A, const float* __restrict__ B, int M, int N, int lda,
                                            int ldb, int m0, int n0, int kbeg, int kend, unsigned char* smem,
                                            f32x4_t (&acc)[BN / 32][BM / 32]) {
  const bool a_vec = (lda % 4 == 0) && (((uintptr_t)A & 15) == 0) && (!A_KC || kend % 4 == 0);
  const bool b_vec = (ldb % 4 == 0) && (((uintptr_t)B & 15) == 0) && (!B_KC || kend % 4 == 0);
  if (a_vec && b_vec) x3_mainloop_v<BM, A_KC, B_KC, BN, true>(A, B, M, N, lda, ldb, m0, n0, kbeg, kend, smem, acc);
  else x3_mainloop_v<BM, A_KC, B_KC, BN, false>(A, B, M, N, lda, ldb, m0, n0, kbeg, kend, smem, acc);
}

template <int ROWS, bool KC>
struct X3TilePc {
  static constexpr int KSTR = 2 * ROWS + 32;
  static constexpr int BYTES = KC ? ROWS * 64 : 32 * KSTR;
};
__device__ __forceinline__ int x3_swz(int row) { return (0x6C >> (((row >> 2) & 3) * 2)) & 3; }

template <int ROWS, bool KC, int NCH>
__device__ __forceinline__ void x3pc_store_tile(unsigned char* hi_base, unsigned char* lo_base, int tid,
                                                const float4 (&in)[NCH]) {
  using T = X3TilePc<ROWS, KC>;
#pragma unroll
  for (int i = 0; i < NCH; ++i) {
    const int q = tid + 256 * i;
    uint32_t h0, l0, h1, l1;
    split_bf16x2(in[i].x, in[i].y, h0, l0);
    split_bf16x2(in[i].z, in[i].w, h1, l1);
    int off;
    if (KC) {
      const int row = q >> 3, c = q & 7;
      off = row * 64 + (((c & 3) ^ x3_swz(row)) * 2 + (c >> 2)) * 8;
    } else {
      constexpr int CPR = ROWS / 4;
      const int kk = q / CPR, row = (q % CPR) * 4;
      off = kk * T::KSTR + row * 2;
    }
    *(uint2*)(hi_base + off) = make_uint2(h0, h1);
    *(uint2*)(lo_base + off) = make_uint2(l0, l1);
  }
}
template <int ROWS, bool KC>
__device__ __forceinline__ bf16x8_t x3pc_frag(const unsigned char* base, int row16, int lane) {
  using T = X3TilePc<ROWS, KC>;
  if (KC) {
    const int row = row16 + (lane & 15);
    const uint4 v = *(const uint4*)(base + row * 64 + (((lane >> 4) ^ x3_swz(row)) * 16));
    return __builtin_bit_cast(bf16x8_t, v);
  } else {
    const int g = lane >> 4, q = (lane >> 2) & 3, pp = lane & 3;
    const unsigned char* p = base + (4 * g + q) * T::KSTR + (row16 + 4 * pp) * 2;
    const uint32_t a0 = (uint32_t)(uintptr_t)((__attribute__((address_space(3))) const unsigned char*)p);
    const x3_s16x4_t lo = __builtin_amdgcn_ds_read_tr16_b64_v4i16((__attribute__((address_space(3))) x3_s16x4_t*)(uintptr_t)a0);
    const x3_s16x4_t hi =
        __builtin_amdgcn_ds_read_tr16_b64_v4i16((__attribute__((address_space(3))) x3_s16x4_t*)(uintptr_t)(a0 + 16 * T::KSTR));
    const x3_s16x8_t v = {lo[0], lo[1], lo[2], lo[3], hi[0], hi[1], hi[2], hi[3]};
    return __builtin_bit_cast(bf16x8_t, v);
  }
}

template <bool A_KC, bool B_KC>
__device__ __forceinline__ void x3_mainloop_pc(const float* __restrict__ A, const float* __restrict__ B, int M, int N, int lda,
                                               int ldb, int m0, int n0, int kbeg, int kend, unsigned char* smem,
                                               f32x4_t (&acc)[4][4]) {
  constexpr int BM = 128, BN = 128, BKx = 32, NCH = 4;
  constexpr int ABYTES = X3TilePc<BM, A_KC>::BYTES, BBYTES = X3TilePc<BN, B_KC>::BYTES;
  constexpr int STAGE = 2 * (ABYTES + BBYTES);
  const int tid = threadIdx.x, lane = tid & 63;
  const int wave = __builtin_amdgcn_readfirstlane(tid >> 6);
  const int nk = ((kend - kbeg + BKx - 1) / BKx + 3) & ~3;
#pragma unroll
  for (int i = 0; i < 4; ++i)
#pragma unroll
    for (int j = 0; j < 4; ++j) acc[i][j] = (f32x4_t){0.f, 0.f, 0.f, 0.f};
  if (wave >= 4) {
    const int pt = tid - 256;
    X3Src<BM, A_KC, NCH, true> sa;
    X3Src<BN, B_KC, NCH, true> sb;
    sa.init(A, lda, m0, M, kbeg, kend, pt);
    sb.init(B, ldb, n0, N, kbeg, kend, pt);
    float4 ar[4][NCH], br[4][NCH];
#pragma unroll
    for (int s = 0; s < 4; ++s) {
      sa.load(kbeg + s * BKx, pt, ar[s]);
      sb.load(kbeg + s * BKx, pt, br[s]);
    }
    auto put = [&](int stage, const float4 (&a)[NCH], const float4 (&b)[NCH]) {
      unsigned char* st = smem + stage * STAGE;
      x3pc_store_tile<BM, A_KC, NCH>(st, st + ABYTES, pt, a);
      x3pc_store_tile<BN, B_KC, NCH>(st + 2 * ABYTES, st + 2 * ABYTES + BBYTES, pt, b);
    };
    put(0, ar[0], br[0]);
    sa.load(kbeg + 4 * BKx, pt, ar[0]);
    sb.load(kbeg + 4 * BKx, pt, br[0]);
    __syncthreads();
    auto step = [&](int kt, auto s_) {
      constexpr int S = decltype(s_)::value;
      put(S & 1, ar[S], br[S]);
      sa.load(kbeg + (kt + 5) * BKx, pt, ar[S]);
      sb.load(kbeg + (kt + 5) * BKx, pt, br[S]);
      __syncthreads();
    };
    for (int kt = 0; kt < nk; kt += 4) {
      step(kt, std::integral_constant<int, 1>());
      step(kt + 1, std::integral_constant<int, 2>());
      step(kt + 2, std::integral_constant<int, 3>());
      step(kt + 3, std::integral_constant<int, 0>());
    }
  } else {
    const int wm = wave >> 1, wn = wave & 1;
    __syncthreads();
    auto step = [&](auto p_) {
      constexpr int P = decltype(p_)::value;
      const unsigned char* st = smem + P * STAGE;
      bf16x8_t bh[4], bl[4], ah[4], al[4];
#pragma unroll
      for (int i = 0; i < 4; ++i) {
        bh[i] = x3pc_frag<BN, B_KC>(st + 2 * ABYTES, wn * 64 + i * 16, lane);
        bl[i] = x3pc_frag<BN, B_KC>(st + 2 * ABYTES + BBYTES, wn * 64 + i * 16, lane);
      }
#pragma unroll
      for (int j = 0; j < 4; ++j) {
        ah[j] = x3pc_frag<BM, A_KC>(st, wm * 64 + j * 16, lane);
        al[j] = x3pc_frag<BM, A_KC>(st + ABYTES, wm * 64 + j * 16, lane);
      }
#pragma unroll
      for (int i = 0; i < 4; ++i)
#pragma unroll
        for (int j = 0; j < 4; ++j) {
          acc[i][j] = __builtin_amdgcn_mfma_f32_16x16x32_bf16(bl[i], ah[j], acc[i][j], 0, 0, 0);
          acc[i][j] = __builtin_amdgcn_mfma_f32_16x16x32_bf16(bh[i], al[j], acc[i][j], 0, 0, 0);
          acc[i][j] = __builtin_amdgcn_mfma_f32_16x16x32_bf16(bh[i], ah[j], acc[i][j], 0, 0, 0);
        }
      __syncthreads();
    };
    for (int kt = 0; kt < nk; kt += 2) {
      step(std::integral_constant<int, 0>());
      step(std::integral_constant<int, 1>());
    }
  }
}

}
```

### include/comic_hip.h

```cpp
#ifndef COMIC_HIP_H_
#define COMIC_HIP_H_

#include <stddef.h>
#include <stdint.h>

#ifdef __cplusplus
extern "C" {
#endif

#define COMIC_F32 0
#define COMIC_BF16 1
#define COMIC_F16 2
#define COMIC_ABI_VERSION 1
#define COMIC_CONV_TILES 61
#define COMIC_WS_TILE 54
#define COMIC_IMG_TILE 55
#define COMIC_CHAIN_TILE 62

const char* comic_last_error(void);
int comic_abi_version(void);
int comic_device_count(void);


int comic_pack_conv_weights(const float* w_hwio, void* w_packed, int kh, int kw, int cin, int cout,
                            int dtype, void* stream);

int comic_fold_bn(const float* beta, const float* mean, const float* var, float eps, float* scale,
                  float* shift, int c, void* stream);

typedef struct comic_cnn_op {
  int32_t kind;
  int32_t src, dst;
  int32_t src_coff, dst_coff;
  int32_t H, W, Cin, Cout, KH, KW, SH, SW, PT, PL, Ho, Wo;
  int32_t weight;
  int32_t relu;
  int32_t out_f32;
  int32_t src_f32;
  int32_t lane;
  int32_t tile;
  int32_t group;
  int32_t flags;
  int32_t min_lds;
} comic_cnn_op;
#define COMIC_OP_RAW 1
#define COMIC_OP_POOLED_SRC 2

#define COMIC_OP_X3 4
#define COMIC_OP_CHAIN_LINK 8
#define COMIC_OP_CHAIN_KEEP 16

typedef struct comic_conv_weight {
  const void* w;
  const float* scale;
  const float* shift;
  const void* w_frag;
} comic_conv_weight;

int comic_cnn_forward(const comic_cnn_op* ops, int n_ops, void* const* buffers,
                      const int32_t* buf_channels, const comic_conv_weight* weights, int batch,
                      int dtype, void* stream);

int comic_cnn_pack_frag_weights(const void* w_plan, void* w_frag, const int64_t* table_dev, int n_weights,
                                int64_t total_elems, void* stream);

long comic_cnn_group_args_bytes(const comic_cnn_op* ops, int n_ops);
int comic_cnn_build_group_args(const comic_cnn_op* ops, int n_ops, void* const* buffers,
                               const int32_t* buf_channels, const comic_conv_weight* weights,
                               int batch, void* host_out);
int comic_cnn_forward_grouped(const comic_cnn_op* ops, int n_ops, void* const* buffers,
                              const int32_t* buf_channels, const comic_conv_weight* weights,
                              int batch, int dtype, const void* group_args_dev, void* stream);

typedef struct comic_image_desc {
  int64_t offset;
  int32_t in_h, in_w;
  int32_t flip, oy, ox;
  float sy, sx;
} comic_image_desc;
int comic_image_preprocess(const uint8_t* blob, const void* desc, int n, float* dst ,
                           int out_h, int out_w, int resize, void* stream);

int comic_jpeg_pixels(const int16_t* coef, const void* infos, int n, int max_blocks, int max_w, int max_h, uint8_t* planes,
                      uint8_t* pixels, void* stream);
int comic_jpeg_preprocess(const int16_t* coef, const void* infos, int n, int max_blocks, uint8_t* planes, const uint8_t* blob,
                          const void* desc, float* dst , int out_h, int out_w, int resize, void* stream);
int comic_jpeg_preprocess_packed(const uint16_t* packed, const void* infos, int n, int max_blocks, uint8_t* planes,
                                 const uint8_t* blob, const void* desc, float* dst , int out_h, int out_w,
                                 int resize, void* stream);

typedef struct comic_conv_grad {
  const float* w_master;
  float* dw;
  float* dbeta;
  void* w_bwd;
  int32_t bwd_tile;
  int32_t reserved;
} comic_conv_grad;
int64_t comic_cnn_backward_scratch_bytes(const comic_cnn_op* ops, int n_ops, int batch, int dtype, int lanes);
int comic_cnn_backward(const comic_cnn_op* ops, int n_ops, void* const* buffers,
                       void* const* grad_buffers, const int32_t* buf_channels,
                       const comic_conv_weight* weights, const comic_conv_grad* grads, int batch,
                       int dtype, int filters_ready ,
                       void* scratch, int64_t scratch_bytes, void* stream, void* wgrad_stream);
#define COMIC_CNN_BWD_NO_ACT_FUSION 2
int comic_cnn_backward_sched(const comic_cnn_op* ops, int n_ops, const int32_t* sched, int n_sched, void* const* buffers,
                             void* const* grad_buffers, void* const* grad_buffers_alt, const int32_t* buf_channels,
                             const comic_conv_weight* weights, const comic_conv_grad* grads, int batch, int dtype,
                             int filters_ready, void* scratch, int64_t scratch_bytes, void* stream0, void* stream1,
                             void* wgrad_stream);
int comic_cnn_pack_x3_weights(const float* const* masters, void* const* outs, const int32_t* cout, const int32_t* taps,
                              const int32_t* cin, int n, void* stream);
int comic_cnn_pack_bwd_filters(const comic_cnn_op* ops, int n_ops, const comic_conv_grad* grads,
                               int dtype, void* stream);
int comic_cnn_refresh_weights(const float* master, void* plan_copy, int64_t n, const float* beta,
                              const float* mean, const float* scale, float* shift,
                              int64_t channels, void* stream);
int comic_cnn_refresh_weights_dtype(const float* master, void* plan_copy, int64_t n, const float* beta,
                                    const float* mean, const float* scale, float* shift,
                                    int64_t channels, int dtype, void* stream);

int comic_conv2d_bn_relu(const comic_cnn_op* op, const void* x, int x_channels, void* y,
                         int y_channels, const comic_conv_weight* wt, int batch, int dtype,
                         void* stream);

int comic_gemm_f32(const float* A, const float* B, float* C, const float* bias, int M, int N, int K,
                   int lda, int ldb, int ldc, int trans_a, int trans_b, float alpha, float beta,
                   void* stream);

int comic_gemm_f32_split3(const float* A, const float* B, float* C, const float* bias, int M, int N,
                          int K, int lda, int ldb, int ldc, int trans_a, int trans_b, float alpha,
                          float beta, void* workspace ,
                          int64_t workspace_bytes, void* stream);

typedef struct comic_gemm_prob {
  const float* A;
  const float* B;
  float* C;
  const float* bias;
  const float* mask;
  int32_t M, N, K, lda, ldb, ldc, ld_mask;
  float alpha, beta, keep;
  int32_t type, ones_a;
} comic_gemm_prob;
int64_t comic_gemm_group_workspace(const comic_gemm_prob* probs, int n);
int comic_gemm_group(const comic_gemm_prob* probs, int n, void* workspace, int64_t workspace_bytes, void* stream);

int64_t comic_gemm_f32_stream_workspace(int R, int Kin, int N);
int comic_gemm_f32_stream(const float* x, const float* W, const float* bias, float* out, int R, int Kin, int N,
                          void* workspace, int64_t workspace_bytes, void* stream);

int comic_gemm_f32_splitk(const float* A, const float* B, float* C, const float* bias, int M, int N,
                          int K, int lda, int ldb, int ldc, int trans_a, int trans_b, float alpha,
                          float beta, void* workspace, int64_t workspace_bytes, void* stream);

int comic_embed_fwd(const float* table, const int32_t* ids, float* out, int rows, int E, int V,
                    void* stream);
int comic_embed_bwd(const int32_t* ids, const float* dout, float* dtable, int rows, int E, int V,
                    void* stream);

int comic_dropout_apply(const float* x, const float* mask, float keep, float* y, int64_t n,
                        void* stream);
int comic_dropout_mask(float* mask, int64_t n, float keep, uint64_t seed, uint64_t offset,
                       void* stream);
int comic_dropout_mask_dev(float* mask, int64_t n, float keep, const uint64_t* seed_dev,
                           uint64_t offset, void* stream);
int comic_dropout_masks4_dev(float* mask, const int64_t* n4, const float* keep4, const uint64_t* seed_dev,
                             void* stream);
int comic_weighted_sum_tb(const float* rows_tb, const float* w_bt, int T, int B, float* out, void* stream);

int comic_lstm_gates_fwd(const float* g, const float* c_prev, const float* h_prev, float* gates_act,
                         float* c_new, float* h_new, float* y, const float* mask_out, float keep_out,
                         const int32_t* lens, int t, float* c_state, float* h_state, int B, int D,
                         void* stream);
int comic_lstm_gates_bwd(const float* gates_act, const float* c_prev, const float* c_new,
                         const float* dy, const float* mask_out, float keep_out, const int32_t* lens,
                         int t, float* dc_state, float* dh_state, float* dg, int B, int D, void* stream);

typedef struct comic_attn_desc {
  int32_t B, M, D, H, Cv;
  int32_t method;
  int32_t prob;
  int32_t tied;
} comic_attn_desc;

int comic_attn_step_fwd(const comic_attn_desc* d, const float* keys, const float* values,
                        const float* q, const float* ln_g, const float* ln_b, const float* v,
                        const float* tau, const float* mask_alpha, float keep_alpha, float* alpha,
                        float* alpha_d, float* ctx, void* stream);
int comic_attn_step_bwd(const comic_attn_desc* d, const float* keys, const float* values,
                        const float* q, const float* ln_g, const float* ln_b, const float* v,
                        const float* tau, const float* alpha, const float* mask_alpha,
                        float keep_alpha, const float* dctx, const float* dmap, float* dq,
                        float* dkeys, float* dvalues, float* pgrad, void* stream);

int comic_xent_fwd_bwd(float* logits, const int32_t* targets_bt, const float* coef_bt,
                       const float* wmask_bt, const int32_t* lens, float* loss_rows, float* dlogits,
                       int32_t* ids_tb, int T, int B, int V, void* stream);

int comic_argmax_rows(const float* x, int32_t* idx, int rows, int V, void* stream);
int comic_beam_step(const float* logits, float* log_probs, int32_t* finished, int64_t* lengths,
                    int32_t* word_ids, int32_t* parent_ids, float* scores, int B, int W, int V,
                    int end_id, void* stream);

int64_t comic_beam_step_dense_workspace(int B, int W, int D, int V);
int comic_beam_step_dense(const float* y, const float* W_o, const float* b_o, float* log_probs, int32_t* finished,
                          int64_t* lengths, int32_t* word_ids, int32_t* parent_ids, float* scores, int B, int W, int D,
                          int V, int end_id, void* workspace, int64_t workspace_bytes, void* stream);
int comic_gather_rows(const float* in, const int32_t* parent, float* out, int rows, int W, int cols,
                      void* stream);
int comic_gather_tree(const int32_t* step_ids, const int32_t* parent_ids, const int32_t* max_len,
                      int32_t* out, int T, int B, int W, int end_id, void* stream);

int comic_adam_tf(float* w, const float* g, float* m, float* v, int64_t n, float lr_t, float beta1,
                  float beta2, float eps, float l2, float gscale, void* stream);
int comic_ln_tanh_fwd(const float* x, const float* gamma, const float* beta, float* y, float* xhat, int B, int C,
                      float eps, void* stream);
int comic_ln_tanh_bwd_rows(const float* dy, const float* y, const float* xhat, float* pgamma, float* pbeta, int B,
                           int C, void* stream);
int comic_momentum_tf(float* w, const float* g, float* accum, int64_t n, float lr, float momentum, float l2,
                      float gscale, void* stream);
int comic_adam_tf_gated(float* w, const float* g, float* m, float* v, int64_t n, float lr_t, float beta1, float beta2,
                        float epsilon, float l2, float gscale, const float* skip_flag, void* stream);
int comic_momentum_tf_gated(float* w, const float* g, float* accum, int64_t n, float lr, float momentum, float l2,
                            float gscale, const float* skip_flag, void* stream);
int comic_clip_by_norm(float* g, const float* w, const int64_t* chunks, int n_chunks, float l2, float gscale,
                       float clip_norm, float* partial, const float* skip_flag, void* stream);
int comic_debug_occupy_cus(int n_workgroups, int microseconds, void* stream);
int comic_colsum(const float* in, float* out, int rows, int cols, float beta, void* stream);
int comic_axpy(float* y, const float* x, float a, int64_t n, void* stream);

typedef struct comic_decoder_desc {
  int32_t D, E, A, V, C, Cg, H, M;
  int32_t Cv;
  int32_t fm_projection;
  int32_t method, prob;
  int32_t context_layer;
  int32_t init_method;
  int32_t start_id, end_id;
  float keep_in, keep_out, keep_alpha;
  float map_loss_scale;
  uint32_t flags;
  float length_penalty_weight;
  int32_t cell;
} comic_decoder_desc;
#define COMIC_CELL_LSTM 0
#define COMIC_CELL_LN_LSTM 1
#define COMIC_CELL_GRU 2
#define COMIC_DEC_NO_PERSIST 1u
#define COMIC_DEC_NO_PERSIST_BWD 2u
#define COMIC_DEC_NO_FUSED_STEP 4u
#define COMIC_DEC_NO_SPLIT_ATTN_BWD 8u
#define COMIC_DEC_ONE_LANE 16u
#define COMIC_DEC_EXACT_GEMM 32u
#define COMIC_DEC_STAMPS 64u
#define COMIC_DEC_PHASE_FWD 512u
#define COMIC_DEC_PHASE_BWD 1024u
#define COMIC_DEC_NO_GROUP_GEMM 2048u
#define COMIC_DEC_INJECT_TIMEOUT 8192u
#define COMIC_DEC_BWD_OWN_ROWS 4096u
#define COMIC_DEC_NO_LSTM_STREAM 256u
#define COMIC_DEC_NO_BEAM_LOGITS 128u

typedef struct comic_decoder_params {
  float *W_init, *K, *b, *W_m, *W_v, *W_q, *v, *ln_g, *ln_b, *tau, *W_a, *W_o, *b_o, *emb;
  float* cell_ln;
  float *K_c, *b_c;
  float* status;
} comic_decoder_params;

int64_t comic_decoder_train_workspace(const comic_decoder_desc* d, int B, int T);
int64_t comic_decoder_infer_workspace(const comic_decoder_desc* d, int rows, int max_steps);

int comic_decoder_train_step(const comic_decoder_desc* d, const comic_decoder_params* p,
                             const comic_decoder_params* grads, const float* fm,
                             const float* im_embed, const int32_t* inputs_bt,
                             const int32_t* targets_bt, const float* wmask_bt, const float* coef_bt,
                             const int32_t* lens, int B, int T, int Tp, const float* mask_init_in,
                             const float* mask_in, const float* mask_out, const float* mask_alpha,
                             float* logits_tb, int32_t* ids_tb, float* attn_hist, float* loss_rows,
                             float* map_loss, float* dfm, float* dim_embed, void* workspace,
                             int64_t workspace_bytes, void* stream);

int comic_decoder_train_path(void);
int comic_decoder_greedy_path(void);
int comic_decoder_beam_path(void);

int comic_decoder_greedy(const comic_decoder_desc* d, const comic_decoder_params* p, const float* fm,
                         const float* im_embed, int B, int max_steps, int32_t* ids_tb,
                         float* logits_tb, float* attn_hist, int32_t* first_eos, void* workspace,
                         int64_t workspace_bytes, void* stream);

int comic_decoder_sample(const comic_decoder_desc* d, const comic_decoder_params* p, const float* fm,
                         const float* im_embed, int B, int max_steps, const float* gumbel_tb, int32_t* ids_tb,
                         float* logits_tb, float* attn_hist, int32_t* first_eos, void* workspace,
                         int64_t workspace_bytes, void* stream);

int comic_decoder_beam(const comic_decoder_desc* d, const comic_decoder_params* p, const float* fm,
                       const float* im_embed, int B, int W, int max_steps, int32_t* step_ids,
                       int32_t* parent_ids, float* scores, int64_t* lengths, int32_t* finished,
                       float* attn_hist, int32_t* steps_executed, void* workspace,
                       int64_t workspace_bytes, void* stream);

typedef struct comic_scorer comic_scorer;
comic_scorer* comic_scorer_create(const char* ngrams_host, const double* counts_host,
                                  int64_t n_entries, double ref_len);
void comic_scorer_destroy(comic_scorer* s);
int comic_scorer_score(const comic_scorer* s, const char* const* hypos_host, int n,
                       const char* const* refs_host, const int32_t* refs_per_host,
                       double* out_cider_host, double* out_bleu_host, int n_threads);

uint32_t comic_crc32c(const void* data_host, size_t n, uint32_t crc);

#ifdef __cplusplus
}
#endif
#endif
```

Before: 39660 images/sec.

## Add 256-row, 8-wave tile form to grouped GEMM with cost-based selection

Adds a third grouped-GEMM kernel form that uses 256-row M tiles with 512 threads (8 waves). The planner prices both the 128-row and 256-row tilings and picks the 256-row form when all operands are vector-aligned and its estimated cost is lower. The goal is to raise data reuse per workgroup and cut the number of work items and split-K slab traffic for the decoder's batched GEMMs. In exchange the new form uses more LDS and gives fewer workgroups, which can leave the device underfilled. An env flag forces the old 128-row path.

```diff
diff --git a/comic-compact-image-captioning-with-attention_amd/_lib.py b/comic-compact-image-captioning-with-attention_amd/_lib.py
--- a/comic-compact-image-captioning-with-attention_amd/_lib.py
+++ b/comic-compact-image-captioning-with-attention_amd/_lib.py
@@ -45,13 +45,14 @@
 DEC_NO_GROUP_GEMM = 2048
 DEC_BWD_OWN_ROWS = 4096
 DEC_INJECT_TIMEOUT = 8192
+DEC_GG_128 = 16384
 CNN_BWD_NO_ACT_FUSION = 2
 _DEC_ENV = (('COMIC_PERSIST', '0', DEC_NO_PERSIST), ('COMIC_PERSIST_BWD', '0', DEC_NO_PERSIST_BWD),
             ('COMIC_FUSED_STEP', '0', DEC_NO_FUSED_STEP), ('COMIC_SPLIT_ATTN_BWD', '0', DEC_NO_SPLIT_ATTN_BWD),
             ('COMIC_GRAD_LANES', '0', DEC_ONE_LANE), ('COMIC_SPLIT3', '0', DEC_EXACT_GEMM),
             ('COMIC_PERSIST_STAMPS', '1', DEC_STAMPS), ('COMIC_BEAM_LOGITS', '0', DEC_NO_BEAM_LOGITS),
             ('COMIC_LSTM_STREAM', '0', DEC_NO_LSTM_STREAM), ('COMIC_GROUP_GEMM', '0', DEC_NO_GROUP_GEMM),
-            ('COMIC_BWD_OWN_ROWS', '1', DEC_BWD_OWN_ROWS))
+            ('COMIC_BWD_OWN_ROWS', '1', DEC_BWD_OWN_ROWS), ('COMIC_GG_256', '0', DEC_GG_128))
 
 
 def decoder_flags_from_env():
@@ -122,6 +123,7 @@
                                       c_float, P, c_int64, P]),
     'comic_gemm_group_workspace': (c_int64, [P, c_int]),
     'comic_gemm_group': (c_int, [P, c_int, P, c_int64, P]),
+    'comic_gemm_group_rows': (c_int, [P, c_int, P, c_int64, P, c_int]),
     'comic_embed_fwd': (c_int, [P, P, P, c_int, c_int, c_int, P]),
     'comic_embed_bwd': (c_int, [P, P, P, c_int, c_int, c_int, P]),
     'comic_dropout_apply': (c_int, [P, P, c_float, P, c_int64, P]),
diff --git a/comic-compact-image-captioning-with-attention_amd/csrc/decoder_exec.hip b/comic-compact-image-captioning-with-attention_amd/csrc/decoder_exec.hip
--- a/comic-compact-image-captioning-with-attention_amd/csrc/decoder_exec.hip
+++ b/comic-compact-image-captioning-with-attention_amd/csrc/decoder_exec.hip
@@ -568,6 +568,7 @@
   int run(void* slab, int64_t slab_cap, unsigned* tickets, hipStream_t st) {
     if (g.n == 0) return 0;
     int target = kGemmGroupTargetItems;
+    g.force_rows = (g_dec_flags & COMIC_DEC_GG_128) ? 128 : 0;
     for (;;) {
       int64_t need = 0;
       int nt = 0;
diff --git a/comic-compact-image-captioning-with-attention_amd/csrc/gemm_group.h b/comic-compact-image-captioning-with-attention_amd/csrc/gemm_group.h
--- a/comic-compact-image-captioning-with-attention_amd/csrc/gemm_group.h
+++ b/comic-compact-image-captioning-with-attention_amd/csrc/gemm_group.h
@@ -26,6 +26,8 @@
   float* slab;
   unsigned* tickets;
   int xcd_chunk;
+  int force_rows;
+  int tile_rows;
 };
 
 int comic_gemm_group_plan(ComicGemmGroup& g, int target_items, int64_t* slab_bytes, int* n_tickets);
diff --git a/comic-compact-image-captioning-with-attention_amd/csrc/gemm_group.hip b/comic-compact-image-captioning-with-attention_amd/csrc/gemm_group.hip
--- a/comic-compact-image-captioning-with-attention_amd/csrc/gemm_group.hip
+++ b/comic-compact-image-captioning-with-attention_amd/csrc/gemm_group.hip
@@ -6,8 +6,12 @@
 namespace {
 
 constexpr int GB = 128;
+constexpr int GB2 = 256;
 constexpr int kGemmGroupSlots = 512;
+constexpr int kGemmGroupSlots8 = 256;
 constexpr int kItemOverhead = 6;
+constexpr int kKtileCost4 = 4, kKtileCost8 = 3;
+enum { GG_FORM_4W = 0, GG_FORM_PC = 1, GG_FORM_8W = 2 };
 constexpr int kSc1 = 16;
 typedef __attribute__((ext_vector_type(4))) unsigned gg_u32x4_t;
 
@@ -25,6 +29,8 @@
 
 constexpr int kGroupLds = 4 * (X3Tile<GB, true>::BYTES + X3Tile<GB, true>::BYTES);
 static_assert(X3Tile<GB, true>::BYTES >= X3Tile<GB, false>::BYTES, "LDS of the k-contiguous form bounds the others");
+constexpr int kGroupLds8 = 4 * (X3Tile<GB2, true>::BYTES + X3Tile<GB, true>::BYTES);
+static_assert(X3Tile<GB2, true>::BYTES >= X3Tile<GB2, false>::BYTES, "LDS of the k-contiguous form bounds the others");
 constexpr int kGroupLdsPc = 2 * 2 * (X3TilePc<GB, false>::BYTES + X3TilePc<GB, false>::BYTES);
 static_assert(X3TilePc<GB, false>::BYTES >= X3TilePc<GB, true>::BYTES, "LDS of the row-contiguous form bounds the others");
 
@@ -49,10 +55,13 @@
   }
 }
 
-template <bool PC>
-__global__ __launch_bounds__(PC ? 512 : 256) void gemm_group_x3_kernel(ComicGemmGroup g) {
-  constexpr int NT = PC ? 512 : 256;
-  constexpr int LDS = PC ? kGroupLdsPc : kGroupLds;
+template <int FORM>
+__global__ __launch_bounds__(FORM == GG_FORM_4W ? 256 : 512) void gemm_group_x3_kernel(ComicGemmGroup g) {
+  constexpr bool PC = FORM == GG_FORM_PC;
+  constexpr int NT = FORM == GG_FORM_4W ? 256 : 512;
+  constexpr int LDS = PC ? kGroupLdsPc : FORM == GG_FORM_8W ? kGroupLds8 : kGroupLds;
+  constexpr int TBM = FORM == GG_FORM_8W ? GB2 : GB;
+  constexpr int WGM = PC ? 2 : NT / 128;
   extern __shared__ __attribute__((aligned(16))) unsigned char smem[];
   int bid = blockIdx.x;
   if (g.xcd_chunk > 0 && bid < g.xcd_chunk * 8) bid = (bid & 7) * g.xcd_chunk + (bid >> 3);
@@ -70,27 +79,28 @@
   const int pw = min(PW, p.tiles_n - panel * PW);
   const int mt = rem / pw, nt = panel * PW + rem % pw;
   const int tile = mt * p.tiles_n + nt;
-  const int m0 = mt * GB, n0 = nt * GB;
+  const int m0 = mt * TBM, n0 = nt * GB;
   const int kbeg = S > 1 ? slice * p.k_per_slice : 0;
   const int kend = S > 1 ? min(p.K, kbeg + p.k_per_slice) : p.K;
   const int tid = threadIdx.x, lane = tid & 63, wave = tid >> 6;
   const int wm = wave >> 1, wn = wave & 1;
+  constexpr int TILE = TBM * GB;
 
   const long tile_id = (long)p.ticket0 + tile;
-  const __amdgpu_buffer_rsrc_t sr = gg_rsrc(g.slab + ((long)p.slab_tile0 + (long)tile * S) * (GB * GB), (long)S * GB * GB * 4);
-  const unsigned sbase = (unsigned)slice * (GB * GB * 4);
+  const __amdgpu_buffer_rsrc_t sr = gg_rsrc(g.slab + ((long)p.slab_tile0 + (long)tile * S) * TILE, (long)S * TILE * 4);
+  const unsigned sbase = (unsigned)slice * (TILE * 4);
   if (p.ones_a) {
-    constexpr int KG = NT / 32;
+    constexpr int KG = 8;
     float4* red = (float4*)smem;
     const int cg = tid & 31, kg = tid >> 5, n = n0 + 4 * cg;
     const bool vec = (p.ldb % 4 == 0) && (((uintptr_t)p.B & 15) == 0);
     float4 sm = make_float4(0.f, 0.f, 0.f, 0.f);
-    if (n < p.N)
+    if (n < p.N && kg < KG)
       for (int k = kbeg + kg; k < kend; k += KG) {
         const float4 v = load4(p.B + (size_t)k * p.ldb + n, p.N - n, vec);
         sm.x += v.x; sm.y += v.y; sm.z += v.z; sm.w += v.w;
       }
-    red[kg * 32 + cg] = sm;
+    if (kg < KG) red[kg * 32 + cg] = sm;
     __syncthreads();
     if (tid < 32) {
       float4 tot = red[cg];
@@ -109,15 +119,22 @@
       if (p.type == COMIC_GG_TN) x3_mainloop_pc<false, false>(p.A, p.B, p.M, p.N, p.lda, p.ldb, m0, n0, kbeg, kend, smem, acc);
       else if (p.type == COMIC_GG_NN) x3_mainloop_pc<true, false>(p.A, p.B, p.M, p.N, p.lda, p.ldb, m0, n0, kbeg, kend, smem, acc);
       else x3_mainloop_pc<true, true>(p.A, p.B, p.M, p.N, p.lda, p.ldb, m0, n0, kbeg, kend, smem, acc);
+    } else if constexpr (FORM == GG_FORM_8W) {
+      if (p.type == COMIC_GG_TN)
+        x3_mainloop_v<TBM, false, false, GB, true, NT>(p.A, p.B, p.M, p.N, p.lda, p.ldb, m0, n0, kbeg, kend, smem, acc);
+      else if (p.type == COMIC_GG_NN)
+        x3_mainloop_v<TBM, true, false, GB, true, NT>(p.A, p.B, p.M, p.N, p.lda, p.ldb, m0, n0, kbeg, kend, smem, acc);
+      else
+        x3_mainloop_v<TBM, true, true, GB, true, NT>(p.A, p.B, p.M, p.N, p.lda, p.ldb, m0, n0, kbeg, kend, smem, acc);
     } else {
       if (p.type == COMIC_GG_TN)
-        x3_mainloop<GB, false, false, GB>(p.A, p.B, p.M, p.N, p.lda, p.ldb, m0, n0, kbeg, kend, smem, acc);
+        x3_mainloop<TBM, false, false, GB, NT>(p.A, p.B, p.M, p.N, p.lda, p.ldb, m0, n0, kbeg, kend, smem, acc);
       else if (p.type == COMIC_GG_NN)
-        x3_mainloop<GB, true, false, GB>(p.A, p.B, p.M, p.N, p.lda, p.ldb, m0, n0, kbeg, kend, smem, acc);
+        x3_mainloop<TBM, true, false, GB, NT>(p.A, p.B, p.M, p.N, p.lda, p.ldb, m0, n0, kbeg, kend, smem, acc);
       else
-        x3_mainloop<GB, true, true, GB>(p.A, p.B, p.M, p.N, p.lda, p.ldb, m0, n0, kbeg, kend, smem, acc);
-    }
-    const bool owner = wave < 4;
+        x3_mainloop<TBM, true, true, GB, NT>(p.A, p.B, p.M, p.N, p.lda, p.ldb, m0, n0, kbeg, kend, smem, acc);
+    }
+    const bool owner = !PC || wave < 4;
     if (S == 1) {
       if (owner)
 #pragma unroll
@@ -146,7 +163,8 @@
   }
   __syncthreads();
   if (!*s_last) return;
-  const int n_chunks = p.ones_a ? 1 : (GB * GB / 4) / NT;
+  const int n_chunks = p.ones_a ? 1 : (TILE / 4) / NT;
+  static_assert((TILE / 4) % (4 * NT) == 0 && WGM * 64 == TBM, "gemm_group: combine chunks / wave rows");
 #pragma unroll 1
   for (int c = 0; c < n_chunks; c += 4) {
     float4 sum[4];
@@ -156,7 +174,7 @@
     for (int s = 0; s < S; ++s) {
       float4 v[4];
 #pragma unroll
-      for (int u = 0; u < 4; ++u) v[u] = gg_load16_sc1(sr, (unsigned)s * (GB * GB * 4) + (unsigned)(tid + NT * (c + u)) * 16u);
+      for (int u = 0; u < 4; ++u) v[u] = gg_load16_sc1(sr, (unsigned)s * (TILE * 4) + (unsigned)(tid + NT * (c + u)) * 16u);
 #pragma unroll
       for (int u = 0; u < 4; ++u) {
         sum[u].x += v[u].x; sum[u].y += v[u].y; sum[u].z += v[u].z; sum[u].w += v[u].w;
@@ -173,8 +191,29 @@
 
 }
 
+namespace {
+bool gg_vec_ok(const ComicGemmProb& p) {
+  if (p.ones_a) return true;
+  const bool a_kc = p.type != COMIC_GG_TN, b_kc = p.type == COMIC_GG_NT;
+  return p.lda % 4 == 0 && p.ldb % 4 == 0 && ((uintptr_t)p.A & 15) == 0 && ((uintptr_t)p.B & 15) == 0 &&
+         (!(a_kc || b_kc) || p.K % 4 == 0);
+}
+int gg_split_of(int kt, long klen) { return (int)std::min<long>(16, std::max<long>(1, (kt + klen / 2) / klen)); }
+long gg_price(const ComicGemmGroup& g, long klen, int rows, int slots, int ktile_cost) {
+  long items = 0, longest = 0;
+  for (int i = 0; i < g.n; ++i) {
+    const ComicGemmProb& p = g.p[i];
+    const int kt = cdiv(p.K, 32), S = gg_split_of(kt, klen);
+    items += (long)cdiv(p.M, rows) * p.tiles_n * S;
+    if (!p.ones_a) longest = std::max<long>(longest, cdiv(kt, S));
+  }
+  return cdiv64(items, slots) * (longest + kItemOverhead) * ktile_cost;
+}
+}
+
 int comic_gemm_group_plan(ComicGemmGroup& g, int target_items, int64_t* slab_bytes, int* n_tickets) {
   COMIC_REQUIRE(g.n > 0 && g.n <= kGemmGroupMax, "gemm_group: %d problems", g.n);
+  COMIC_REQUIRE(g.force_rows == 0 || g.force_rows == GB || g.force_rows == GB2, "gemm_group: tile rows %d", g.force_rows);
   long cost = 0;
   for (int i = 0; i < g.n; ++i) {
     ComicGemmProb& p = g.p[i];
@@ -184,36 +223,36 @@
     COMIC_REQUIRE(p.ldc >= p.N && (!p.mask || p.ld_mask >= p.N), "gemm_group: leading dimension of problem %d", i);
     if (!p.ones_a) COMIC_REQUIRE(p.lda >= (p.type == COMIC_GG_TN ? p.M : p.K), "gemm_group: lda of problem %d", i);
     COMIC_REQUIRE(p.ldb >= (p.type == COMIC_GG_NT ? p.K : p.N), "gemm_group: ldb of problem %d", i);
-    p.tiles_m = cdiv(p.M, GB);
     p.tiles_n = cdiv(p.N, GB);
     cost += (long)cdiv(p.M, GB) * p.tiles_n * cdiv(p.K, 32);
   }
-  auto split_of = [](int kt, long klen) { return (int)std::min<long>(16, std::max<long>(1, (kt + klen / 2) / klen)); };
-  long klen = std::max<long>(8, cost / std::max(1, target_items));
+  long klen = std::max<long>(8, cost / std::max(1, target_items)), est4 = -1;
   {
-    long best = -1, best_klen = klen, kt_max = 8;
+    long kt_max = 8;
     for (int i = 0; i < g.n; ++i) kt_max = std::max<long>(kt_max, cdiv(g.p[i].K, 32));
-    for (long kl = klen; kl <= kt_max; ++kl) {
-      long items = 0, longest = 0;
-      for (int i = 0; i < g.n; ++i) {
-        const ComicGemmProb& p = g.p[i];
-        const int kt = cdiv(p.K, 32), S = split_of(kt, kl);
-        items += (long)p.tiles_m * p.tiles_n * S;
-        if (!p.ones_a) longest = std::max<long>(longest, cdiv(kt, S));
-      }
-      const long est = cdiv64(items, kGemmGroupSlots) * (longest + kItemOverhead);
-      if (best < 0 || est < best) {
-        best = est;
-        best_klen = kl;
-      }
-    }
-    klen = best_klen;
-  }
+    const long kl0 = klen;
+    for (long kl = kl0; kl <= kt_max; ++kl) {
+      const long est = gg_price(g, kl, GB, kGemmGroupSlots, kKtileCost4);
+      if (est4 < 0 || est < est4) {
+        est4 = est;
+        klen = kl;
+      }
+    }
+  }
+  long items4 = 0;
+  for (int i = 0; i < g.n; ++i) items4 += (long)cdiv(g.p[i].M, GB) * g.p[i].tiles_n * gg_split_of(cdiv(g.p[i].K, 32), klen);
+  const long est8 = items4 > kGemmGroupSlots8 ? gg_price(g, klen, GB2, kGemmGroupSlots8, kKtileCost8) : est4;
+  bool vec = true;
+  for (int i = 0; i < g.n; ++i) vec = vec && gg_vec_ok(g.p[i]);
+  COMIC_REQUIRE(vec || g.force_rows != GB2, "gemm_group: the 256-row form needs 16-byte aligned operand rows");
+  const int rows = g.force_rows ? g.force_rows : (vec && est8 < est4) ? GB2 : GB;
+  g.tile_rows = rows;
   int wg = 0, tickets = 0, slab_tiles = 0;
   for (int i = 0; i < g.n; ++i) {
     ComicGemmProb& p = g.p[i];
-    const int nt = cdiv(p.M, GB) * p.tiles_n, kt = cdiv(p.K, 32);
-    int S = split_of(kt, klen);
+    p.tiles_m = cdiv(p.M, rows);
+    const int nt = p.tiles_m * p.tiles_n, kt = cdiv(p.K, 32);
+    int S = gg_split_of(kt, klen);
     p.k_per_slice = cdiv(kt, S) * 32;
     S = cdiv(p.K, p.k_per_slice);
     p.S = S;
@@ -226,7 +265,7 @@
       tickets += nt;
     }
   }
-  if (slab_bytes) *slab_bytes = (int64_t)slab_tiles * GB * GB * 4;
+  if (slab_bytes) *slab_bytes = (int64_t)slab_tiles * rows * GB * 4;
   if (n_tickets) *n_tickets = tickets;
   return wg;
 }
@@ -235,25 +274,23 @@
   ComicGemmGroup g = g_in;
   g.xcd_chunk = n_wg / 8;
   COMIC_REQUIRE(n_wg > 0, "gemm_group: empty launch");
-  bool pc = n_wg <= 256;
-  for (int i = 0; i < g.n && pc; ++i) {
-    const ComicGemmProb& p = g.p[i];
-    if (p.ones_a) continue;
-    const bool a_kc = p.type != COMIC_GG_TN, b_kc = p.type == COMIC_GG_NT;
-    pc = p.lda % 4 == 0 && p.ldb % 4 == 0 && ((uintptr_t)p.A & 15) == 0 && ((uintptr_t)p.B & 15) == 0 &&
-         (!(a_kc || b_kc) || p.K % 4 == 0);
-  }
-  static PerDeviceOnce once, once_pc;
-  bool& done = pc ? once_pc.slot() : once.slot();
-  const int lds = pc ? kGroupLdsPc : kGroupLds;
+  COMIC_REQUIRE(g.tile_rows == GB || g.tile_rows == GB2, "gemm_group: launch without a plan");
+  bool pc = g.tile_rows == GB && n_wg <= 256;
+  for (int i = 0; i < g.n && pc; ++i) pc = gg_vec_ok(g.p[i]);
+  const int form = g.tile_rows == GB2 ? GG_FORM_8W : pc ? GG_FORM_PC : GG_FORM_4W;
+  static PerDeviceOnce once[3];
+  bool& done = once[form].slot();
+  const int lds = form == GG_FORM_8W ? kGroupLds8 : pc ? kGroupLdsPc : kGroupLds;
+  const void* fns[3] = {(const void*)gemm_group_x3_kernel<GG_FORM_4W>, (const void*)gemm_group_x3_kernel<GG_FORM_PC>,
+                        (const void*)gemm_group_x3_kernel<GG_FORM_8W>};
   if (!done) {
-    const void* fn = pc ? (const void*)gemm_group_x3_kernel<true> : (const void*)gemm_group_x3_kernel<false>;
-    COMIC_REQUIRE(hipFuncSetAttribute(fn, hipFuncAttributeMaxDynamicSharedMemorySize, lds) == hipSuccess,
+    COMIC_REQUIRE(hipFuncSetAttribute(fns[form], hipFuncAttributeMaxDynamicSharedMemorySize, lds) == hipSuccess,
                   "gemm_group: cannot reserve %d bytes of LDS", lds);
     done = true;
   }
-  if (pc) hipLaunchKernelGGL(gemm_group_x3_kernel<true>, dim3((unsigned)n_wg), dim3(512), lds, st, g);
-  else hipLaunchKernelGGL(gemm_group_x3_kernel<false>, dim3((unsigned)n_wg), dim3(256), lds, st, g);
+  if (form == GG_FORM_8W) hipLaunchKernelGGL(gemm_group_x3_kernel<GG_FORM_8W>, dim3((unsigned)n_wg), dim3(512), lds, st, g);
+  else if (pc) hipLaunchKernelGGL(gemm_group_x3_kernel<GG_FORM_PC>, dim3((unsigned)n_wg), dim3(512), lds, st, g);
+  else hipLaunchKernelGGL(gemm_group_x3_kernel<GG_FORM_4W>, dim3((unsigned)n_wg), dim3(256), lds, st, g);
   COMIC_LAUNCH_CHECK("gemm_group");
   return 0;
 }
@@ -278,15 +315,23 @@
 extern "C" int64_t comic_gemm_group_workspace(const comic_gemm_prob* probs, int n) {
   ComicGemmGroup g;
   if (gg_from_public(probs, n, g)) return -1;
-  int64_t slab = 0;
-  int nt = 0;
-  if (comic_gemm_group_plan(g, kPublicTarget, &slab, &nt) < 0) return -1;
-  return slab + 256 + (int64_t)nt * 4;
-}
-
-extern "C" int comic_gemm_group(const comic_gemm_prob* probs, int n, void* workspace, int64_t workspace_bytes, void* stream) {
+  int64_t need = 0;
+  for (int rows : {GB, GB2}) {
+    g.force_rows = rows;
+    int64_t slab = 0;
+    int nt = 0;
+    if (comic_gemm_group_plan(g, kPublicTarget, &slab, &nt) < 0) return -1;
+    need = std::max<int64_t>(need, slab + 256 + (int64_t)nt * 4);
+  }
+  return need;
+}
+
+extern "C" int comic_gemm_group_rows(const comic_gemm_prob* probs, int n, void* workspace, int64_t workspace_bytes, void* stream,
+                                     int tile_rows) {
   ComicGemmGroup g;
   if (int rc = gg_from_public(probs, n, g)) return rc;
+  COMIC_REQUIRE(tile_rows == 0 || tile_rows == GB || tile_rows == GB2, "gemm_group: tile rows %d (0, 128 or 256)", tile_rows);
+  g.force_rows = tile_rows;
   int64_t slab = 0;
   int nt = 0;
   const int wg = comic_gemm_group_plan(g, kPublicTarget, &slab, &nt);
@@ -298,3 +343,7 @@
   if (nt) COMIC_REQUIRE(hipMemsetAsync(g.tickets, 0, (size_t)nt * 4, (hipStream_t)stream) == hipSuccess, "gemm_group: memset");
   return comic_gemm_group_launch(g, wg, (hipStream_t)stream);
 }
+
+extern "C" int comic_gemm_group(const comic_gemm_prob* probs, int n, void* workspace, int64_t workspace_bytes, void* stream) {
+  return comic_gemm_group_rows(probs, n, workspace, workspace_bytes, stream, 0);
+}
diff --git a/comic-compact-image-captioning-with-attention_amd/csrc/gemm_x3_dev.h b/comic-compact-image-captioning-with-attention_amd/csrc/gemm_x3_dev.h
--- a/comic-compact-image-captioning-with-attention_amd/csrc/gemm_x3_dev.h
+++ b/comic-compact-image-captioning-with-attention_amd/csrc/gemm_x3_dev.h
@@ -42,14 +42,14 @@
     base = (size_t)min(k, K - 1) * ld;
   }
 }
-template <int ROWS, bool KC, int NCH, bool VEC>
+template <int ROWS, bool KC, int NCH, bool VEC, int NT = 256>
 __device__ __forceinline__ void x3_load_tile(const float* __restrict__ g, int ld, int row0, int rows_total, int k0, int K,
                                              int tid, float4 (&out)[NCH]) {
 #pragma unroll
   for (int i = 0; i < NCH; ++i) {
     int c, ext, nv;
     size_t base;
-    x3_chunk<ROWS, KC>(tid + 256 * i, ld, row0, rows_total, k0, K, c, ext, nv, base);
+    x3_chunk<ROWS, KC>(tid + NT * i, ld, row0, rows_total, k0, K, c, ext, nv, base);
     const float* bp = g + base;
     if (VEC) {
       out[i] = *(const float4*)(bp + max(0, min(c, ext - 4)));
@@ -59,13 +59,13 @@
     }
   }
 }
-template <int ROWS, bool KC, int NCH, bool VEC>
+template <int ROWS, bool KC, int NCH, bool VEC, int NT = 256>
 __device__ __forceinline__ void x3_mask_tile(int row0, int rows_total, int k0, int K, int tid, float4 (&v)[NCH]) {
 #pragma unroll
   for (int i = 0; i < NCH; ++i) {
     int c, ext, nv;
     size_t base;
-    x3_chunk<ROWS, KC>(tid + 256 * i, 0, row0, rows_total, k0, K, c, ext, nv, base);
+    x3_chunk<ROWS, KC>(tid + NT * i, 0, row0, rows_total, k0, K, c, ext, nv, base);
     if (VEC) {
       const bool ok = nv >= 4;
       v[i].x = ok ? v[i].x : 0.f; v[i].y = ok ? v[i].y : 0.f; v[i].z = ok ? v[i].z : 0.f; v[i].w = ok ? v[i].w : 0.f;
@@ -74,13 +74,13 @@
     }
   }
 }
-template <int ROWS, bool KC, int NCH>
+template <int ROWS, bool KC, int NCH, int NT = 256>
 __device__ __forceinline__ void x3_store_tile(unsigned char* hi_base, unsigned char* lo_base, int tid,
                                               const float4 (&in)[NCH]) {
   using T = X3Tile<ROWS, KC>;
 #pragma unroll
   for (int i = 0; i < NCH; ++i) {
-    const int q = tid + 256 * i;
+    const int q = tid + NT * i;
     uint32_t h0, l0, h1, l1;
     split_bf16x2(in[i].x, in[i].y, h0, l0);
     split_bf16x2(in[i].z, in[i].w, h1, l1);
@@ -119,7 +119,7 @@
 
 
 constexpr unsigned kOor = 0x80000000u;
-template <int ROWS, bool KC, int NCH, bool VEC>
+template <int ROWS, bool KC, int NCH, bool VEC, int NT = 256>
 struct X3Src {
   const float* g;
   int ld, row0, rows_total, kend;
@@ -136,7 +136,7 @@
         kc = (tid & 7) * 4;
 #pragma unroll
         for (int i = 0; i < NCH; ++i) {
-          const int r = row0 + (tid >> 3) + 32 * i;
+          const int r = row0 + (tid >> 3) + (NT / 8) * i;
           rb[i] = r < rows_total ? (unsigned)(((long)r * ld + kc) * 4) : kOor;
         }
       } else {
@@ -145,7 +145,7 @@
         const long rec = ((long)(kend - 1) * ld + min(ld, (rows_total + 3) & ~3)) * 4;
         rs = __builtin_amdgcn_make_buffer_rsrc((void*)g, 0, (int)rec, 0x00020000);
         base = r < rows_total ? (unsigned)(((long)(kbeg + tid / CPR) * ld + r) * 4) : kOor;
-        step8 = (unsigned)((256 / CPR) * ld * 4);
+        step8 = (unsigned)((NT / CPR) * ld * 4);
       }
     }
   }
@@ -160,7 +160,7 @@
           const u4 v = __builtin_amdgcn_raw_buffer_load_b128(rs, (int)o, 0, 0);
           out[i] = make_float4(__uint_as_float(v.x), __uint_as_float(v.y), __uint_as_float(v.z), __uint_as_float(v.w));
         }
-      } else if constexpr (256 % (ROWS / 4) == 0) {
+      } else if constexpr (NT % (ROWS / 4) == 0) {
 #pragma unroll
         for (int i = 0; i < NCH; ++i) {
           const u4 v = __builtin_amdgcn_raw_buffer_load_b128(rs, (int)(base + (unsigned)i * step8), 0, 0);
@@ -171,28 +171,29 @@
         constexpr int CPR = ROWS / 4;
 #pragma unroll
         for (int i = 0; i < NCH; ++i) {
-          const int q = tid + 256 * i, r = row0 + (q % CPR) * 4;
+          const int q = tid + NT * i, r = row0 + (q % CPR) * 4;
           const unsigned o = r < rows_total ? (unsigned)(((long)(k0 + q / CPR) * ld + r) * 4) : kOor;
           const u4 v = __builtin_amdgcn_raw_buffer_load_b128(rs, (int)o, 0, 0);
           out[i] = make_float4(__uint_as_float(v.x), __uint_as_float(v.y), __uint_as_float(v.z), __uint_as_float(v.w));
         }
       }
     } else {
-      x3_load_tile<ROWS, KC, NCH, false>(g, ld, row0, rows_total, k0, kend, tid, out);
+      x3_load_tile<ROWS, KC, NCH, false, NT>(g, ld, row0, rows_total, k0, kend, tid, out);
     }
   }
   __device__ __forceinline__ void mask(int k0, int tid, float4 (&v)[NCH]) {
-    if (!VEC) x3_mask_tile<ROWS, KC, NCH, false>(row0, rows_total, k0, kend, tid, v);
+    if (!VEC) x3_mask_tile<ROWS, KC, NCH, false, NT>(row0, rows_total, k0, kend, tid, v);
   }
 };
 
-template <int BM, bool A_KC, bool B_KC, int BN, bool VEC>
+template <int BM, bool A_KC, bool B_KC, int BN, bool VEC, int NT = 256>
 __device__ __forceinline__ void x3_mainloop_v(const float* __restrict__ A, const float* __restrict__ B, int M, int N, int lda,
                                             int ldb, int m0, int n0, int kbeg, int kend, unsigned char* smem,
-                                            f32x4_t (&acc)[BN / 32][BM / 32]) {
-  constexpr int BKx = 32;
-  constexpr int TM = BM / 32, TN = BN / 32;
-  constexpr int ACH = BM * BKx / 4 / 256, BCH = BN * BKx / 4 / 256;
+                                            f32x4_t (&acc)[BN / 32][BM / (NT / 8)]) {
+  constexpr int BKx = 32, WGM = NT / 128;
+  constexpr int TM = BM / (16 * WGM), TN = BN / 32;
+  constexpr int ACH = BM * BKx / 4 / NT, BCH = BN * BKx / 4 / NT;
+  static_assert(ACH * NT * 4 == BM * BKx && BCH * NT * 4 == BN * BKx && TM >= 1, "x3_mainloop_v: tile / thread count");
   constexpr int ABYTES = X3Tile<BM, A_KC>::BYTES, BBYTES = X3Tile<BN, B_KC>::BYTES;
   unsigned char* Ah = smem;
   unsigned char* Al = Ah + 2 * ABYTES;
@@ -206,8 +207,8 @@
     for (int j = 0; j < TM; ++j) acc[i][j] = (f32x4_t){0.f, 0.f, 0.f, 0.f};
   float4 ar[2][ACH], br[2][BCH];
   const int nk = ((kend - kbeg + BKx - 1) / BKx + 1) & ~1;
-  X3Src<BM, A_KC, ACH, VEC> sa;
-  X3Src<BN, B_KC, BCH, VEC> sb;
+  X3Src<BM, A_KC, ACH, VEC, NT> sa;
+  X3Src<BN, B_KC, BCH, VEC, NT> sb;
   sa.init(A, lda, m0, M, kbeg, kend, tid);
   sb.init(B, ldb, n0, N, kbeg, kend, tid);
   sa.load(kbeg, tid, ar[0]);
@@ -216,8 +217,8 @@
   sb.load(kbeg + BKx, tid, br[1]);
   sa.mask(kbeg, tid, ar[0]);
   sb.mask(kbeg, tid, br[0]);
-  x3_store_tile<BM, A_KC, ACH>(Ah, Al, tid, ar[0]);
-  x3_store_tile<BN, B_KC, BCH>(Bh, Bl, tid, br[0]);
+  x3_store_tile<BM, A_KC, ACH, NT>(Ah, Al, tid, ar[0]);
+  x3_store_tile<BN, B_KC, BCH, NT>(Bh, Bl, tid, br[0]);
   __syncthreads();
   auto step = [&](const int kt, auto par) {
     constexpr int P = decltype(par)::value;
@@ -231,8 +232,8 @@
     }
 #pragma unroll
     for (int j = 0; j < TM; ++j) {
-      ah[j] = x3_frag<BM, A_KC>(Ah + P * ABYTES, wm * (BM / 2) + j * 16, lane);
-      al[j] = x3_frag<BM, A_KC>(Al + P * ABYTES, wm * (BM / 2) + j * 16, lane);
+      ah[j] = x3_frag<BM, A_KC>(Ah + P * ABYTES, wm * (BM / WGM) + j * 16, lane);
+      al[j] = x3_frag<BM, A_KC>(Al + P * ABYTES, wm * (BM / WGM) + j * 16, lane);
     }
 #pragma unroll
     for (int i = 0; i < TN; ++i)
@@ -244,8 +245,8 @@
       }
     sa.mask(kbeg + (kt + 1) * BKx, tid, ar[P ^ 1]);
     sb.mask(kbeg + (kt + 1) * BKx, tid, br[P ^ 1]);
-    x3_store_tile<BM, A_KC, ACH>(Ah + (P ^ 1) * ABYTES, Al + (P ^ 1) * ABYTES, tid, ar[P ^ 1]);
-    x3_store_tile<BN, B_KC, BCH>(Bh + (P ^ 1) * BBYTES, Bl + (P ^ 1) * BBYTES, tid, br[P ^ 1]);
+    x3_store_tile<BM, A_KC, ACH, NT>(Ah + (P ^ 1) * ABYTES, Al + (P ^ 1) * ABYTES, tid, ar[P ^ 1]);
+    x3_store_tile<BN, B_KC, BCH, NT>(Bh + (P ^ 1) * BBYTES, Bl + (P ^ 1) * BBYTES, tid, br[P ^ 1]);
 #ifdef COMIC_X3_SCHED
     __builtin_amdgcn_sched_group_barrier(0x020, ACH + BCH, 0);
     __builtin_amdgcn_sched_group_barrier(0x100, 64, 0);
@@ -264,14 +265,14 @@
   }
 }
 
-template <int BM, bool A_KC, bool B_KC, int BN>
+template <int BM, bool A_KC, bool B_KC, int BN, int NT = 256>
 __device__ __forceinline__ void x3_mainloop(const float* __restrict__ A, const float* __restrict__ B, int M, int N, int lda,
                                             int ldb, int m0, int n0, int kbeg, int kend, unsigned char* smem,
-                                            f32x4_t (&acc)[BN / 32][BM / 32]) {
+                                            f32x4_t (&acc)[BN / 32][BM / (NT / 8)]) {
   const bool a_vec = (lda % 4 == 0) && (((uintptr_t)A & 15) == 0) && (!A_KC || kend % 4 == 0);
   const bool b_vec = (ldb % 4 == 0) && (((uintptr_t)B & 15) == 0) && (!B_KC || kend % 4 == 0);
-  if (a_vec && b_vec) x3_mainloop_v<BM, A_KC, B_KC, BN, true>(A, B, M, N, lda, ldb, m0, n0, kbeg, kend, smem, acc);
-  else x3_mainloop_v<BM, A_KC, B_KC, BN, false>(A, B, M, N, lda, ldb, m0, n0, kbeg, kend, smem, acc);
+  if (a_vec && b_vec) x3_mainloop_v<BM, A_KC, B_KC, BN, true, NT>(A, B, M, N, lda, ldb, m0, n0, kbeg, kend, smem, acc);
+  else x3_mainloop_v<BM, A_KC, B_KC, BN, false, NT>(A, B, M, N, lda, ldb, m0, n0, kbeg, kend, smem, acc);
 }
 
 template <int ROWS, bool KC>
diff --git a/include/comic_hip.h b/include/comic_hip.h
--- a/include/comic_hip.h
+++ b/include/comic_hip.h
@@ -145,6 +145,8 @@
 } comic_gemm_prob;
 int64_t comic_gemm_group_workspace(const comic_gemm_prob* probs, int n);
 int comic_gemm_group(const comic_gemm_prob* probs, int n, void* workspace, int64_t workspace_bytes, void* stream);
+int comic_gemm_group_rows(const comic_gemm_prob* probs, int n, void* workspace, int64_t workspace_bytes, void* stream,
+                          int tile_rows);
 
 int64_t comic_gemm_f32_stream_workspace(int R, int Kin, int N);
 int comic_gemm_f32_stream(const float* x, const float* W, const float* bias, float* out, int R, int Kin, int N,
@@ -258,6 +260,7 @@
 #define COMIC_DEC_PHASE_BWD 1024u
 #define COMIC_DEC_NO_GROUP_GEMM 2048u
 #define COMIC_DEC_INJECT_TIMEOUT 8192u
+#define COMIC_DEC_GG_128 16384u
 #define COMIC_DEC_BWD_OWN_ROWS 4096u
 #define COMIC_DEC_NO_LSTM_STREAM 256u
 #define COMIC_DEC_NO_BEAM_LOGITS 128u
```

Measured after the change: 39690 images/sec, median of 5. About the same (+0.1%).
